# pabloconrat/our_first_climate_model

Hardware: NVIDIA B200
Metric: column*wavelength*layer flux updates/s (repwvl-100 RCE step) (higher is better)
Workload: dtype f64

## Files before the change

### our_first_climate_model_b200/csrc/rcm_capi.cu

```cuda
#include <algorithm>
#include <cmath>
#include <cstdio>
#include <cstdlib>
#include <cstring>
#include <new>
#include <functional>
#include <string>
#include <vector>

#include "rcm_jac.cuh"
#include "rcm_fdh.cuh"

#ifndef M_PI
#define M_PI 3.14159265358979323846
#endif

struct rcm_solver {
    int device = 0;
    cudaStream_t own_stream = nullptr, stream = nullptr;
    rcm_params p{};
    DevConst dc{};
    bool const_dirty = true;
    int opt_angle_cubes = 1;
    int opt_angle_pairs = 1;
    int opt_config = 0;
    int opt_stage_rows = 1;
    int opt_path = 0;
    int opt_cplk_narrow = 0;
    double tau_clamp = 240.0;
    double T_floor = 0.0;
    int clampk = 1;
    bool has_table = false, has_spectral = false;
    std::vector<double> p_grid, t_ref, t_pert, wvl, weight;
    double* d_coef3 = nullptr;
    double *d_xsec_file = nullptr, *d_coef = nullptr, *d_planck_c = nullptr, *d_planck_k = nullptr, *d_exp_tab = nullptr;
    int* d_species = nullptr;
    bool coef_dirty = true;
    int ncol = 0, cap = 0, nactive = 0, h2o_slot = -1;
    int species[RCM_NSPECIES]{};
    bool has_plevel = false;
    double plevel[RCM_NLEVEL]{};
    double *d_T = nullptr, *d_Ts = nullptr, *d_vmr = nullptr, *d_rh = nullptr, *d_Tprev = nullptr;
    float* d_time = nullptr;
    double *d_Ed = nullptr, *d_Eu = nullptr, *d_dE = nullptr, *d_dt = nullptr;
    double *d_diag = nullptr, *d_scalars = nullptr, *d_tau = nullptr, *d_red = nullptr;
    int* d_lowpos = nullptr;
    unsigned* d_ticket = nullptr;
    double *d_solar_col = nullptr, *d_cloud_col = nullptr;
    bool has_col_solar = false, has_col_cloud = false;
    size_t diag_steps = 0, tau_cap = 0;
    long step_index = 0;
    bool tau_valid = false;
    bool lbl_mode = false;
    int lbl_nwvl = 0;
    double lbl_co2_factor = 1.0;
    bool lbl_has_o3_ref = false;
    double *d_lbl_lo = nullptr, *d_lbl_hi = nullptr, *d_lbl_tau5 = nullptr, *d_lbl_h2o_ref = nullptr,
           *d_lbl_o3_ref = nullptr, *d_sH = nullptr, *d_sO = nullptr, *d_dTstat = nullptr, *d_part = nullptr;
    size_t part_cap = 0;
    unsigned char* d_tile = nullptr;
    double* d_spart = nullptr;
    unsigned* d_counter = nullptr;
    unsigned* d_multi = nullptr;
    size_t multi_cap = 0;
    int opt_multi = 1;
    size_t tile_cap = 0, spart_cap = 0;
    bool tile_vmr_valid = false;
    std::vector<double> stage;
    std::string err;
    long launches = 0;
    std::vector<std::pair<cudaEvent_t, cudaEvent_t>> ev_free, ev_used;
    cudaStream_t pipe_stream[3] = {nullptr, nullptr, nullptr};
    cudaEvent_t pipe_done[3] = {nullptr, nullptr, nullptr}, pipe_start = nullptr;
    struct HostGraph {
        cudaGraphExec_t exec = nullptr;
        SplitArgs sig{};
        const void* host[7] = {};
        const void* dev[4] = {};
        double dT_converged = 0.0;
        int ncol = 0, nchunk = 0, nkernels = 0;
        long captures = 0, replays = 0;
        bool failed = false;
    } hg;
    cudaStream_t sp_up = nullptr, sp_rt[2] = {nullptr, nullptr}, sp_down = nullptr;
    cudaEvent_t sp_prep[24] = {}, sp_rtdone[24] = {}, sp_end = nullptr;
    double kt_ms = 0.0;
    long kt_n = 0;
    unsigned char* d_diagnose = nullptr;
    size_t diagnose_bytes = 0;
    cudaStream_t dg_stream[2] = {nullptr, nullptr};
    cudaEvent_t dg_fork = nullptr, dg_join[2] = {nullptr, nullptr};
    int* h_fdh_count = nullptr;
};

namespace {

int fail(rcm_solver* s, int code, const std::string& msg) {
    if (s) s->err = msg;
    return code;
}

int cuda_fail(rcm_solver* s, cudaError_t e, const char* what) {
    return fail(s, RCM_ERR_CUDA, std::string(what) + ": " + cudaGetErrorString(e));
}

#define CU(call)                                          \
    do {                                                  \
        cudaError_t e__ = (call);                         \
        if (e__ != cudaSuccess) return cuda_fail(s, e__, #call); \
    } while (0)

template <class T>
cudaError_t dalloc(T*& p, size_t n) {
    if (p) cudaFree(p);
    p = nullptr;
    return cudaMalloc((void**)&p, n * sizeof(T));
}

void set_active_species(rcm_solver* s) {
    s->nactive = 0;
    s->h2o_slot = -1;
    for (int k = 0; k < RCM_NSPECIES; ++k)
        if (s->p.species_mask & (1u << k)) {
            if (k == 0) s->h2o_slot = s->nactive;
            s->species[s->nactive++] = k;
        }
}

void build_angles(rcm_solver* s) {
    DevConst& d = s->dc;
    const int na = s->p.nangle;
    const double dmu = 1.0 / (double)na;
    d.nangle = na;
    std::vector<std::vector<int>> chains;
    struct PairUnit { int type; double inv_mu_root; std::vector<int> a, b; };
    std::vector<PairUnit> pairs;
    if (s->opt_angle_cubes) {
        std::vector<char> used(na, 0);
        for (int i = na - 1; i >= 0; --i) {
            if (used[i]) continue;
            std::vector<int> ch;
            for (int n = 2 * i + 1;; n /= 3) {
                used[(n - 1) / 2] = 1;
                ch.push_back((n - 1) / 2);
                if (n % 3 != 0) break;
            }
            chains.push_back(ch);
        }
        if (s->opt_angle_pairs) {
            struct Edge { int ca, cb, type, R; };
            std::vector<Edge> edges;
            const int pa_[3] = {3, 5, 3}, pb_[3] = {5, 7, 7};
            for (size_t x = 0; x < chains.size(); ++x)
                for (size_t y = 0; y < chains.size(); ++y) {
                    const int a = 2 * chains[x][0] + 1, b = 2 * chains[y][0] + 1;
                    for (int t = 0; t < 3; ++t)
                        if (a > b && pa_[t] * a == pb_[t] * b) edges.push_back({(int)x, (int)y, t, pa_[t] * a});
                }
            std::vector<int> best, cur;
            std::vector<char> taken(chains.size(), 0);
            std::function<void(size_t)> rec = [&](size_t e) {
                if (cur.size() > best.size()) best = cur;
                if (e >= edges.size() || cur.size() + (edges.size() - e) <= best.size() || edges.size() > 24) return;
                if (!taken[edges[e].ca] && !taken[edges[e].cb]) {
                    taken[edges[e].ca] = taken[edges[e].cb] = 1;
                    cur.push_back((int)e);
                    rec(e + 1);
                    cur.pop_back();
                    taken[edges[e].ca] = taken[edges[e].cb] = 0;
                }
                rec(e + 1);
            };
            rec(0);
            if (best.size() > (size_t)MAX_PAIR) best.resize(MAX_PAIR);
            std::vector<char> gone(chains.size(), 0);
            for (int e : best) {
                const Edge& ed = edges[e];
                pairs.push_back({ed.type, 2.0 * na / (double)ed.R, chains[ed.ca], chains[ed.cb]});
                gone[ed.ca] = gone[ed.cb] = 1;
            }
            std::vector<std::vector<int>> rest;
            for (size_t x = 0; x < chains.size(); ++x)
                if (!gone[x]) rest.push_back(chains[x]);
            chains.swap(rest);
        }
    } else {
        for (int i = 0; i < na; ++i) chains.push_back({i});
    }
    if (chains.size() % 2) chains.push_back({-1});
    d.nchain = (int)chains.size();
    double sum = 0.0, x_max = 0.0, x_min = 1e300;
    int slot = 0;
    for (int a = 0; a < MAX_ANGLE + 2; ++a) {
        d.chain_len[a] = 1;
        d.neg_inv_mu_l2e[a] = 0.0;
        d.cmu[a] = 0.0;
    }
    auto node_mu = [&](int i) { return dmu / 2.0 + dmu * (double)i; };
    d.npair = (int)pairs.size();
    for (int p = 0; p <= MAX_PAIR; ++p) d.pair_nim[p] = 0.0;
    for (int p = 0; p < d.npair; ++p) {
        d.pair_type[p] = pairs[p].type;
        d.pair_lenA[p] = (int)pairs[p].a.size();
        d.pair_lenB[p] = (int)pairs[p].b.size();
        d.pair_nim[p] = -pairs[p].inv_mu_root * EXP_L2E;
        x_max = std::max(x_max, pairs[p].inv_mu_root);
        for (const std::vector<int>* ch : {&pairs[p].a, &pairs[p].b})
            for (int i : *ch) {
                const double mu = node_mu(i);
                d.cmu[slot] = 2 * M_PI * mu * dmu;
                sum += d.cmu[slot++];
                x_min = std::min(x_min, 1.0 / mu);
            }
    }
    for (int ic = 0; ic < d.nchain; ++ic) {
        d.chain_len[ic] = (int)chains[ic].size();
        for (size_t m = 0; m < chains[ic].size(); ++m, ++slot) {
            if (chains[ic][m] < 0) continue;
            const double mu = node_mu(chains[ic][m]);
            d.cmu[slot] = 2 * M_PI * mu * dmu;
            sum += d.cmu[slot];
            if (m == 0) {
                d.neg_inv_mu_l2e[ic] = (-1.0 / mu) * EXP_L2E;
                x_max = std::max(x_max, 1.0 / mu);
            }
            x_min = std::min(x_min, 1.0 / mu);
        }
    }
    d.pair_nim[d.npair] = d.neg_inv_mu_l2e[0];
    d.nslot = slot;
    d.csum = sum;
    {
        const double ec7[4] = {0x1.62e42fefa3685p-8, 0x1.ebfbdff82c58fp-17, 0x1.c6b09b1799fcbp-26, 0x1.3b2ab6fba4e77p-35};
        const double ec10[4] = {0x1.62e42fefa39efp-11, 0x1.ebfbe033445b4p-23, 0x1.c6b08d704a0c0p-35, 0.0};
        for (int k = 0; k < 4; ++k) d.expc[k] = (EXP_LOG2 == 7) ? ec7[k] : ec10[k];
#ifdef RCM_EXP_DEG_OVERRIDE
        {
            const double c = 0.6931471805599453 / EXP_TAB;
            const double tay[4] = {c, c * c / 2, c * c * c / 6, c * c * c * c / 24};
            for (int k = 0; k < 4; ++k) d.expc[k] = (k <= EXP_DEG) ? tay[k] : 0.0;
        }
#endif
    }
    s->tau_clamp = 999.0 * 0.6931471805599453 / x_max;
    s->clampk = (s->tau_clamp * x_min > 92.2) ? 0 : 1;
}

const rcm_solver* g_const_owner[64] = {nullptr};

int refresh_const(rcm_solver* s) {
    const int dev = s->device & 63;
    if (g_const_owner[dev] != s) {
        CU(cudaDeviceSynchronize());
        s->const_dirty = true;
        g_const_owner[dev] = s;
    }
    if (!s->const_dirty) return RCM_OK;
    CU(cudaStreamSynchronize(s->stream));
    DevConst& d = s->dc;
    set_active_species(s);
    d.nactive = s->nactive;
    for (int k = 0; k < RCM_NSPECIES; ++k) d.species[k] = (k < s->nactive) ? s->species[k] : 0;
    d.cloud_layer = s->p.cloud_layer;
    d.cloud_row = s->p.cloud_layer < 0 ? -1 : (s->p.cloud_layer < HALF ? s->p.cloud_layer : 29 - s->p.cloud_layer);
    d.cloud_tau = s->p.cloud_tau;
    for (int r = 0; r < RCM_NLAYER; ++r) d.cloud_w[r] = (r == d.cloud_row) ? 1.0 : 0.0;
    d.dp = s->p.dp;
    d.max_dT = s->p.max_dT;
    d.dt_cap = s->p.dt_cap;
    d.solar_irr = s->p.solar_irr;
    d.dT_converged = s->p.dT_converged;
    build_angles(s);
    if (s->has_table && s->has_plevel) {
        const double avog = 6.02214076e23, molMassAir = 0.0289647, earthAccel = 9.80665;
        double P[RCM_NLEVEL];
        for (int k = 0; k < RCM_NLEVEL; ++k) P[k] = s->plevel[RCM_NLEVEL - 1 - k] * 100.0;
        for (int k = 0; k < RCM_NLAYER; ++k) {
            const int l = RCM_NLAYER - 1 - k;
            const int r = l < HALF ? l : 29 - l;
            const double midP = (P[k + 1] + P[k]) / 2;
            const long ip = rcm_lowerpos_impl(s->p_grid.data(), (int)s->p_grid.size(), midP);
            d.ip[l] = (int)ip;
            d.ipcell[r] = r * (d.n_tpert - 1);
            d.delP[r] = (midP - s->p_grid[ip]) / (s->p_grid[ip + 1] - s->p_grid[ip]);
            d.numDens[r] = (P[k] - P[k + 1]) * avog / molMassAir / earthAccel;
            d.tref_ip[r] = s->t_ref[ip];
        }
    }
    if (s->has_plevel) {
        for (int l = 0; l < RCM_NLAYER; ++l) {
            d.player[l] = (s->plevel[l] + s->plevel[l + 1]) / 2.0;
            d.conv[l] = std::pow(1000.0 / d.player[l], 2.0 / 7.0);
        }
    }
    cudaError_t e = rcm_upload_const(d);
    if (e != cudaSuccess) return cuda_fail(s, e, "upload constants");
    if (s->has_table && s->has_plevel && s->coef_dirty) {
        const size_t n = (size_t)RCM_NLAYER * (d.n_tpert - 1) * d.nwvl * s->nactive * 4;
        CU(dalloc(s->d_coef, n));
        CU(dalloc(s->d_species, (size_t)RCM_NSPECIES));
        CU(cudaMemcpyAsync(s->d_species, s->species, sizeof(s->species), cudaMemcpyHostToDevice, s->stream));
        CU(rcm_launch_coef(s->d_xsec_file, s->d_coef, d.n_tpert, d.n_species, d.nwvl, d.n_p, s->nactive, s->d_species,
                           s->stream));
        if (s->nactive == 5) {
            const size_t nrows = (size_t)RCM_NLAYER * (d.n_tpert - 1) * d.nwvl;
            CU(dalloc(s->d_coef3, nrows * 16));
            CU(rcm_launch_coef3(s->d_coef, s->d_coef3, nrows, s->stream));
            s->launches += 1;
        }
        CU(cudaStreamSynchronize(s->stream));
        s->launches += 1;
        s->coef_dirty = false;
    }
    s->const_dirty = false;
    return RCM_OK;
}

int ensure_columns(rcm_solver* s, int ncol) {
    if (ncol <= s->cap && s->d_T) return RCM_OK;
    const size_t n = (size_t)ncol;
    CU(dalloc(s->d_T, n * NLAY));
    CU(dalloc(s->d_Ts, n));
    CU(dalloc(s->d_vmr, n * RCM_NSPECIES * NLAY));
    CU(dalloc(s->d_rh, n * NLAY));
    CU(dalloc(s->d_Tprev, n * NLAY));
    CU(dalloc(s->d_time, n));
    CU(dalloc(s->d_Ed, n * NLEV));
    CU(dalloc(s->d_Eu, n * NLEV));
    CU(dalloc(s->d_dE, n * NLAY));
    CU(dalloc(s->d_dt, n));
    CU(dalloc(s->d_lowpos, n * NLAY));
    s->cap = ncol;
    s->diag_steps = 0;
    s->part_cap = 0;
    s->tile_cap = s->spart_cap = 0;
    s->tile_vmr_valid = false;
    if (s->d_dTstat) cudaFree(s->d_dTstat);
    s->d_dTstat = nullptr;
    if (s->d_solar_col) cudaFree(s->d_solar_col);
    if (s->d_cloud_col) cudaFree(s->d_cloud_col);
    s->d_solar_col = s->d_cloud_col = nullptr;
    s->has_col_solar = s->has_col_cloud = false;
    return RCM_OK;
}

int ensure_diag(rcm_solver* s, int nsteps) {
    if ((size_t)nsteps <= s->diag_steps && s->d_diag) return RCM_OK;
    CU(dalloc(s->d_diag, (size_t)nsteps * s->cap * 4));
    CU(dalloc(s->d_scalars, (size_t)nsteps * 4));
    CU(dalloc(s->d_red, rcm_reduce_scratch_doubles(nsteps)));
    CU(dalloc(s->d_ticket, (size_t)nsteps));
    CU(cudaMemsetAsync(s->d_ticket, 0, (size_t)nsteps * sizeof(unsigned), s->stream));
    s->diag_steps = nsteps;
    return RCM_OK;
}

int ensure_tau(rcm_solver* s) {
    const size_t need = (size_t)s->ncol * s->dc.nwvl * NLAY;
    if (need <= s->tau_cap && s->d_tau) return RCM_OK;
    CU(dalloc(s->d_tau, need));
    s->tau_cap = need;
    return RCM_OK;
}

struct CtaShape { int C, nthreads, per_sm; double eff; };
const CtaShape kShapes[] = {{16, 128, 3, 1.0}, {8, 128, 3, 0.95}, {4, 128, 3, 0.89}, {32, 192, 2, 0.9}, {16, 96, 4, 0.93}};
constexpr int kAutoShapes = 3;

struct Part { int col0, ncols; CtaShape sh; };

double part_cost(const CtaShape& sh, int ncols, int nwvl, int nsm) {
    if (ncols <= 0) return 0.0;
    const long tiles = (ncols + sh.C - 1) / sh.C, slots = (long)nsm * sh.per_sm;
    const long rounds = (tiles + slots - 1) / slots;
    const int G = sh.nthreads / (2 * sh.C);
    return (double)rounds * ((nwvl + G - 1) / G) / sh.eff;
}

int plan_parts(const rcm_solver* s, int ncol, int nsm, Part* parts) {
    if (s->opt_config > 0 && s->opt_config <= 5) {
        parts[0] = {0, ncol, kShapes[s->opt_config - 1]};
        return 1;
    }
    const int nwvl = s->dc.nwvl;
    CtaShape best = kShapes[0];
    for (int k = 1; k < kAutoShapes; ++k)
        if (part_cost(kShapes[k], ncol, nwvl, nsm) < part_cost(best, ncol, nwvl, nsm)) best = kShapes[k];
    parts[0] = {0, ncol, best};
    return 1;
}

int nsm_of(const rcm_solver* s) {
    int nsm = 148;
    cudaDeviceGetAttribute(&nsm, cudaDevAttrMultiProcessorCount, s->device);
    return nsm;
}

int launch_part(rcm_solver* s, int mode, int nsteps, bool want_diag, const Part& p, int nsm, cudaStream_t st) {
    const size_t o = (size_t)p.col0;
    StepArgs a{};
    a.ncol = p.ncols;
    a.diag_ncol = s->ncol;
    a.C = p.sh.C;
    a.ntiles = (p.ncols + a.C - 1) / a.C;
    a.nthreads = p.sh.nthreads;
    a.clampk = s->clampk;
    a.stage_rows = s->opt_stage_rows;
    a.tau_clamp = s->tau_clamp;
    a.T_floor = s->T_floor;
    a.nsteps = nsteps;
    a.step_index = s->step_index;
    a.coef = s->d_coef;
    a.planck_c = s->d_planck_c;
    a.planck_k = s->d_planck_k;
    a.Tlayer = s->d_T + o * NLAY;
    a.Tsurf = s->d_Ts + o;
    a.vmr = s->d_vmr + o * s->nactive * NLAY;
    a.rel_hum = s->d_rh + o * NLAY;
    a.Tprev = s->d_Tprev + o * NLAY;
    a.time_h = s->d_time + o;
    a.E_down = s->d_Ed + o * NLEV;
    a.E_up = s->d_Eu + o * NLEV;
    a.dE = s->d_dE + o * NLAY;
    a.dt = s->d_dt + o;
    a.diag = want_diag ? s->d_diag + o * 4 : nullptr;
    a.tau_io = s->d_tau ? s->d_tau + o * s->dc.nwvl * NLAY : nullptr;
    a.lowpos_t = s->d_lowpos + o * NLAY;
    a.exp_tab = s->d_exp_tab;
    a.h2o_slot = s->h2o_slot;
    a.solar_col = s->has_col_solar ? s->d_solar_col + o : nullptr;
    a.cloud_col = s->has_col_cloud ? s->d_cloud_col + o : nullptr;
    int per_sm = p.sh.per_sm;
    if (rcm_step_smem_bytes(a.C, s->nactive, a.nthreads) * per_sm > 224 * 1024) per_sm = 1;
    if (const char* e = std::getenv("RCM_CTAS_PER_SM")) {
        const int v = std::atoi(e);
        if (v >= 1 && v < per_sm) per_sm = v;
    }
    const int ctas = nsm * per_sm;
    const int grid = a.ntiles < ctas ? a.ntiles : ctas;
    CU(rcm_launch_step(mode, a, s->nactive, grid, st));
    s->launches += 1;
    return RCM_OK;
}


bool use_split(const rcm_solver* s) {
    return !s->lbl_mode && s->has_table && s->nactive == 5 && s->opt_config == 0 && s->opt_path == 0;
}

struct SplitGeom { int ntiles, nitem, nsplit; };
SplitGeom split_geom(const rcm_solver* s, int ncols) {
    SplitGeom g;
    g.ntiles = (ncols + 15) / 16;
    g.nitem = (s->dc.nwvl + 3) / 4;
    g.nsplit = (g.nitem + rcm_split_ipu() - 1) / rcm_split_ipu();
    return g;
}

int ensure_split(rcm_solver* s) {
    const SplitGeom g = split_geom(s, s->cap);
    const size_t tiles = (size_t)g.ntiles, need_part = tiles * g.nsplit * rcm_split_part_doubles();
    if (tiles > s->tile_cap || !s->d_tile) {
        CU(dalloc(s->d_tile, tiles * rcm_split_tile_bytes()));
        s->tile_cap = tiles;
        s->tile_vmr_valid = false;
    }
    if (need_part > s->spart_cap || !s->d_spart) {
        CU(dalloc(s->d_spart, need_part));
        s->spart_cap = need_part;
    }
    if (tiles > s->multi_cap || !s->d_multi) {
        if (s->d_multi) CU(cudaFree(s->d_multi));
        s->d_multi = nullptr;
        CU(cudaMalloc((void**)&s->d_multi, 2 * tiles * sizeof(unsigned)));
        s->multi_cap = tiles;
    }
    if (!s->d_dTstat) CU(dalloc(s->d_dTstat, (size_t)s->cap));
    if (!s->d_counter) {
        CU(dalloc(s->d_counter, (size_t)4));
        CU(cudaMemsetAsync(s->d_counter, 0, 4 * sizeof(unsigned), s->stream));
    }
    return RCM_OK;
}

SplitArgs split_args(rcm_solver* s, int col0, int ncols, int which) {
    const SplitGeom g = split_geom(s, ncols);
    const size_t o = (size_t)col0, t0 = o / 16;
    SplitArgs a{};
    a.ncol = ncols;
    a.diag_ncol = s->ncol;
    a.ntiles = g.ntiles;
    a.nsplit = g.nsplit;
    a.ipu = rcm_split_ipu();
    a.nitem = g.nitem;
    a.nunits = g.ntiles * g.nsplit;
    a.stage_rows = s->opt_stage_rows;
    a.clampk = s->clampk;
    a.h2o_slot = s->h2o_slot;
    a.tau_clamp = s->tau_clamp;
    a.T_floor = s->T_floor;
    a.coef = s->d_coef3;
    a.planck_c = s->d_planck_c;
    a.planck_k = s->d_planck_k;
    a.exp_tab = s->d_exp_tab;
    a.Tlayer = s->d_T + o * NLAY;
    a.Tsurf = s->d_Ts + o;
    a.vmr = s->d_vmr + o * s->nactive * NLAY;
    a.rel_hum = s->d_rh + o * NLAY;
    a.Tprev = s->d_Tprev + o * NLAY;
    a.time_h = s->d_time + o;
    a.E_down = s->d_Ed + o * NLEV;
    a.E_up = s->d_Eu + o * NLEV;
    a.dE = s->d_dE + o * NLAY;
    a.dt = s->d_dt + o;
    a.diag = s->d_diag + o * 4;
    a.solar_col = s->has_col_solar ? s->d_solar_col + o : nullptr;
    a.cloud_col = s->has_col_cloud ? s->d_cloud_col + o : nullptr;
    a.tile = s->d_tile + t0 * rcm_split_tile_bytes();
    a.part = s->d_spart + t0 * g.nsplit * rcm_split_part_doubles();
    a.dTstat = s->d_dTstat + o;
    a.counter = s->d_counter + which;
    a.quota = 1 << 30;
    return a;
}

int split_grid(const rcm_solver* s, const SplitArgs& a, int nsm) {
    (void)s;
    if (a.quota < a.nunits) return (a.nunits + a.quota - 1) / a.quota;
    int per_sm = 3;
    if (const char* e = std::getenv("RCM_CTAS_PER_SM")) {
        const int v = std::atoi(e);
        if (v >= 1 && v < per_sm) per_sm = v;
    }
    return std::min(a.nunits, nsm * per_sm);
}

int split_rt(rcm_solver* s, const SplitArgs& a, int nsm, cudaStream_t st, bool timed) {
    std::pair<cudaEvent_t, cudaEvent_t> ev{};
    if (timed) {
        if (!s->ev_free.empty()) {
            ev = s->ev_free.back();
            s->ev_free.pop_back();
        } else {
            CU(cudaEventCreate(&ev.first));
            CU(cudaEventCreate(&ev.second));
        }
        CU(cudaEventRecord(ev.first, st));
    }
    CU(rcm_launch_split_rt(a, split_grid(s, a, nsm), st));
    s->launches += 1;
    if (timed) {
        CU(cudaEventRecord(ev.second, st));
        s->ev_used.push_back(ev);
        if (s->ev_used.size() >= 1024) {
            const int rc = rcm_kernel_time_ms(s, 0, nullptr, nullptr);
            if (rc != RCM_OK) return rc;
        }
    }
    return RCM_OK;
}

int split_advance(rcm_solver* s, int nsteps) {
    int st = refresh_const(s);
    if (st != RCM_OK) return st;
    st = ensure_split(s);
    if (st != RCM_OK) return st;
    const int nsm = nsm_of(s);
    const SplitArgs a = split_args(s, 0, s->ncol, 0);
    SplitColFlags f{};
    f.prep = 1;
    f.first = (s->step_index == 0);
    f.write_all_vmr = !s->tile_vmr_valid;
    CU(rcm_launch_split_col(a, f, s->stream));
    s->launches += 1;
    s->tile_vmr_valid = true;
    static const int multi_rounds = std::getenv("RCM_MULTI_ROUNDS") ? std::atoi(std::getenv("RCM_MULTI_ROUNDS")) : 24;
    const int grid1 = split_grid(s, a, nsm);
    const bool few_rounds = a.nunits < (long long)multi_rounds * grid1;
    const bool fits = (long long)a.nunits * nsteps + 2LL * grid1 < (1LL << 31);
    if (nsteps >= 2 && fits && (s->opt_multi == 2 || (s->opt_multi == 1 && few_rounds))) {
        SplitMultiArgs m{};
        m.nsteps = nsteps;
        m.done = s->d_multi;
        m.ready = s->d_multi + a.ntiles;
        CU(cudaMemsetAsync(s->d_multi, 0, 2 * (size_t)a.ntiles * sizeof(unsigned), s->stream));
        SplitArgs am = a;
        am.quota = 1 << 30;
        CU(rcm_launch_split_multi(am, m, split_grid(s, am, nsm), s->stream));
        s->launches += 1;
        return RCM_OK;
    }
    for (int k = 0; k < nsteps; ++k) {
        st = split_rt(s, a, nsm, s->stream, k < 4);
        if (st != RCM_OK) return st;
        SplitColFlags e{};
        e.finish = 1;
        e.prep = (k + 1 < nsteps);
        e.first = 0;
        e.write_out = (k + 1 == nsteps);
        e.diag_step = k;
        CU(rcm_launch_split_col(a, e, s->stream));
        s->launches += 1;
    }
    return RCM_OK;
}

int launch(rcm_solver* s, int mode, int nsteps, bool want_diag) {
    int st = refresh_const(s);
    if (st != RCM_OK) return st;
    if (mode == MODE_RT ? !s->has_spectral : !s->has_table) return fail(s, RCM_ERR_STATE, "no lookup table loaded");
    if (s->ncol <= 0) return fail(s, RCM_ERR_STATE, "no columns loaded");
    const int nsm = nsm_of(s);
    Part parts[2];
    const int nparts = plan_parts(s, s->ncol, nsm, parts);
    std::pair<cudaEvent_t, cudaEvent_t> ev;
    if (!s->ev_free.empty()) {
        ev = s->ev_free.back();
        s->ev_free.pop_back();
    } else {
        CU(cudaEventCreate(&ev.first));
        CU(cudaEventCreate(&ev.second));
    }
    CU(cudaEventRecord(ev.first, s->stream));
    for (int ip = 0; ip < nparts; ++ip) {
        st = launch_part(s, mode, nsteps, want_diag, parts[ip], nsm, s->stream);
        if (st != RCM_OK) return st;
    }
    CU(cudaEventRecord(ev.second, s->stream));
    if (mode == MODE_STEP) s->ev_used.push_back(ev); else s->ev_free.push_back(ev);
    if (s->ev_used.size() >= 1024) {
        st = rcm_kernel_time_ms(s, 0, nullptr, nullptr);
        if (st != RCM_OK) return st;
    }
    return RCM_OK;
}


int step_host_split(rcm_solver* s, int nchunk, const double* Tlayer_in, const double* Tsurf_in, const double* vmr_active_in,
                    double* E_down, double* E_up, double* dE, double* Tlayer_out, double* Tsurf_out) {
    int st = ensure_split(s);
    if (st != RCM_OK) return st;
    if (!s->sp_up) {
        int lo = 0, hi = 0;
        CU(cudaDeviceGetStreamPriorityRange(&lo, &hi));
        CU(cudaStreamCreateWithPriority(&s->sp_up, cudaStreamNonBlocking, hi));
        CU(cudaStreamCreateWithPriority(&s->sp_down, cudaStreamNonBlocking, hi));
        for (int i = 0; i < 2; ++i) CU(cudaStreamCreateWithPriority(&s->sp_rt[i], cudaStreamNonBlocking, lo));
        for (int i = 0; i < 24; ++i) {
            CU(cudaEventCreateWithFlags(&s->sp_prep[i], cudaEventDisableTiming));
            CU(cudaEventCreateWithFlags(&s->sp_rtdone[i], cudaEventDisableTiming));
        }
        CU(cudaEventCreateWithFlags(&s->sp_end, cudaEventDisableTiming));
    }
    const int nsm = nsm_of(s);
    const int per = ((s->ncol + nchunk - 1) / nchunk + 15) / 16 * 16;
    int bounds[24];
    int nb = 0;
    bounds[nb++] = 0;
    if (nchunk >= 4 && per >= 64) {
        const int q = per / 4 / 16 * 16;
        bounds[nb++] = q;
        for (int c0 = per; c0 < s->ncol - q; c0 += per) bounds[nb++] = c0;
        bounds[nb++] = std::max(bounds[nb - 1], s->ncol - q) / 16 * 16;
    } else {
        for (int c0 = per; c0 < s->ncol; c0 += per) bounds[nb++] = c0;
    }
    bounds[nb] = s->ncol;
    const size_t D = sizeof(double);
    const int na = s->nactive;
    auto enqueue = [&](bool timed) -> int {
    int nk = 0;
    CU(cudaEventRecord(s->sp_end, s->stream));
    for (cudaStream_t q : {s->sp_up, s->sp_rt[0], s->sp_rt[1], s->sp_down}) CU(cudaStreamWaitEvent(q, s->sp_end, 0));
    for (int k = 0; k < nb; ++k) {
        const int c0 = bounds[k], n = bounds[k + 1] - c0;
        if (n <= 0) continue;
        const size_t o = (size_t)c0;
        cudaStream_t q = s->sp_up;
        if (Tlayer_in) CU(cudaMemcpyAsync(s->d_T + o * NLAY, Tlayer_in + o * NLAY, n * NLAY * D, cudaMemcpyHostToDevice, q));
        if (Tsurf_in) CU(cudaMemcpyAsync(s->d_Ts + o, Tsurf_in + o, n * D, cudaMemcpyHostToDevice, q));
        if (vmr_active_in)
            CU(cudaMemcpyAsync(s->d_vmr + o * na * NLAY, vmr_active_in + o * na * NLAY, (size_t)n * na * NLAY * D,
                               cudaMemcpyHostToDevice, q));
        SplitArgs a = split_args(s, c0, n, 1 + k % 2);
        a.quota = 4;
        SplitArgs ac = a;
        ac.counter = nullptr;
        SplitColFlags f{};
        f.prep = 1;
        f.first = (s->step_index == 0);
        f.write_all_vmr = !s->tile_vmr_valid || vmr_active_in != nullptr;
        CU(rcm_launch_split_col(ac, f, q));
        CU(cudaEventRecord(s->sp_prep[k], q));
        q = s->sp_rt[k % 2];
        CU(cudaStreamWaitEvent(q, s->sp_prep[k], 0));
        CU(cudaMemsetAsync(a.counter, 0, sizeof(unsigned), q));
        st = split_rt(s, a, nsm, q, timed);
        if (st != RCM_OK) return st;
        nk += 3;
        CU(cudaEventRecord(s->sp_rtdone[k], q));
        q = s->sp_down;
        CU(cudaStreamWaitEvent(q, s->sp_rtdone[k], 0));
        SplitColFlags e{};
        e.finish = 1;
        e.write_out = 1;
        CU(rcm_launch_split_col(ac, e, q));
        s->launches += 2;
        if (E_down) CU(cudaMemcpyAsync(E_down + o * NLEV, s->d_Ed + o * NLEV, n * NLEV * D, cudaMemcpyDeviceToHost, q));
        if (E_up) CU(cudaMemcpyAsync(E_up + o * NLEV, s->d_Eu + o * NLEV, n * NLEV * D, cudaMemcpyDeviceToHost, q));
        if (dE) CU(cudaMemcpyAsync(dE + o * NLAY, s->d_dE + o * NLAY, n * NLAY * D, cudaMemcpyDeviceToHost, q));
        if (Tlayer_out) CU(cudaMemcpyAsync(Tlayer_out + o * NLAY, s->d_T + o * NLAY, n * NLAY * D, cudaMemcpyDeviceToHost, q));
        if (Tsurf_out) CU(cudaMemcpyAsync(Tsurf_out + o, s->d_Ts + o, n * D, cudaMemcpyDeviceToHost, q));
    }
    CU(cudaEventRecord(s->sp_end, s->sp_down));
    CU(cudaStreamWaitEvent(s->stream, s->sp_end, 0));
    CU(rcm_launch_reduce_diag(s->d_diag, 1, s->ncol, s->p.dT_converged, s->d_red, s->d_ticket, s->d_scalars, s->stream));
    s->launches += 1;
    s->hg.nkernels = nk + 1;
    return RCM_OK;
    };

    const bool steady = s->step_index > 0 && s->tile_vmr_valid && !vmr_active_in && !s->hg.failed && !std::getenv("RCM_NO_GRAPH");
    bool launched = false;
    if (steady) {
        rcm_solver::HostGraph& g = s->hg;
        const SplitArgs sig = split_args(s, 0, s->ncol, 1);
        const void* host[7] = {Tlayer_in, Tsurf_in, E_down, E_up, dE, Tlayer_out, Tsurf_out};
        const void* dev[4] = {s->d_diag, s->d_red, s->d_ticket, s->d_scalars};
        const bool same = g.exec && std::memcmp(&g.sig, &sig, sizeof(sig)) == 0 && std::memcmp(g.host, host, sizeof(host)) == 0 &&
                          std::memcmp(g.dev, dev, sizeof(dev)) == 0 && g.dT_converged == s->p.dT_converged && g.ncol == s->ncol &&
                          g.nchunk == nchunk;
        if (!same) {
            if (g.exec) cudaGraphExecDestroy(g.exec);
            g.exec = nullptr;
            cudaGraph_t graph = nullptr;
            const long launches0 = s->launches;
            bool ok = true;
            for (const void* hp : host) {
                cudaPointerAttributes at{};
                if (hp && (cudaPointerGetAttributes(&at, hp) != cudaSuccess || at.type != cudaMemoryTypeHost)) ok = false;
            }
            cudaGetLastError();
            ok = ok && cudaStreamBeginCapture(s->stream, cudaStreamCaptureModeRelaxed) == cudaSuccess;
            if (ok) {
                ok = enqueue(false) == RCM_OK;
                ok = (cudaStreamEndCapture(s->stream, &graph) == cudaSuccess) && ok && graph;
            }
            s->launches = launches0;
            g.captures += 1;
            if (ok) ok = cudaGraphInstantiate(&g.exec, graph, 0) == cudaSuccess;
            if (graph) cudaGraphDestroy(graph);
            if (!ok) {
                cudaGetLastError();
                g.exec = nullptr;
                bool pinned = true;
                for (const void* hp : host) {
                    cudaPointerAttributes at{};
                    if (hp && (cudaPointerGetAttributes(&at, hp) != cudaSuccess || at.type != cudaMemoryTypeHost)) pinned = false;
                }
                cudaGetLastError();
                if (pinned) g.failed = true;
            } else {
                g.sig = sig;
                std::memcpy(g.host, host, sizeof(host));
                std::memcpy(g.dev, dev, sizeof(dev));
                g.dT_converged = s->p.dT_converged;
                g.ncol = s->ncol;
                g.nchunk = nchunk;
            }
        }
        if (g.exec) {
            CU(cudaGraphLaunch(g.exec, s->stream));
            s->launches += g.nkernels;
            g.replays += 1;
            launched = true;
        }
    }
    if (!launched) {
        st = enqueue(true);
        if (st != RCM_OK) return st;
    }
    s->step_index += 1;
    s->tau_valid = false;
    s->tile_vmr_valid = true;
    CU(cudaStreamSynchronize(s->stream));
    return RCM_OK;
}

}

extern "C" {

int rcm_device_count(void) {
    int n = 0;
    if (cudaGetDeviceCount(&n) != cudaSuccess) return 0;
    return n;
}

int rcm_create(int device, const rcm_params* p, rcm_solver** out) {
    if (!out) return RCM_ERR_ARG;
    *out = nullptr;
    int n = 0;
    if (cudaGetDeviceCount(&n) != cudaSuccess || n <= 0) return RCM_ERR_NO_DEVICE;
    if (device < 0 || device >= n) return RCM_ERR_ARG;
    rcm_solver* s = new (std::nothrow) rcm_solver();
    if (!s) return RCM_ERR_NOMEM;
    s->device = device;
    if (p) s->p = *p; else rcm_default_params(&s->p);
    if (s->p.nangle < 1 || s->p.nangle > MAX_ANGLE || s->p.cloud_layer >= RCM_NLAYER) {
        delete s;
        return RCM_ERR_ARG;
    }
    if (cudaSetDevice(device) != cudaSuccess || cudaStreamCreateWithFlags(&s->own_stream, cudaStreamNonBlocking) != cudaSuccess) {
        delete s;
        return RCM_ERR_CUDA;
    }
    s->stream = s->own_stream;
    double tab[EXP_TAB];
    for (int j = 0; j < EXP_TAB; ++j) {
        const double v = std::exp2((double)j / EXP_TAB);
        unsigned long long bits;
        std::memcpy(&bits, &v, 8);
        bits -= (unsigned long long)j << (20 - EXP_LOG2 + 32);
        std::memcpy(&tab[j], &bits, 8);
    }
    if (dalloc(s->d_exp_tab, EXP_TAB) != cudaSuccess ||
        cudaMemcpy(s->d_exp_tab, tab, sizeof(tab), cudaMemcpyHostToDevice) != cudaSuccess) {
        delete s;
        return RCM_ERR_CUDA;
    }
    set_active_species(s);
    *out = s;
    return RCM_OK;
}

int rcm_destroy(rcm_solver* s) {
    if (!s) return RCM_OK;
    cudaSetDevice(s->device);
    cudaStreamSynchronize(s->stream);
    if (g_const_owner[s->device & 63] == s) g_const_owner[s->device & 63] = nullptr;
    void* ptrs[] = {s->d_coef3, s->d_xsec_file, s->d_coef, s->d_species, s->d_planck_c, s->d_planck_k, s->d_exp_tab, s->d_T, s->d_Ts, s->d_vmr, s->d_rh,
                    s->d_Tprev, s->d_time, s->d_lbl_lo, s->d_lbl_hi, s->d_lbl_tau5, s->d_lbl_h2o_ref, s->d_lbl_o3_ref, s->d_sH, s->d_sO,
                    s->d_dTstat, s->d_part, s->d_Ed, s->d_Eu, s->d_dE, s->d_dt, s->d_diag, s->d_scalars, s->d_red, s->d_tau,
                    s->d_lowpos, s->d_solar_col, s->d_cloud_col, s->d_ticket, s->d_tile, s->d_spart, s->d_counter, s->d_multi, s->d_diagnose};
    for (void* q : ptrs)
        if (q) cudaFree(q);
    for (auto& e : s->ev_free) { cudaEventDestroy(e.first); cudaEventDestroy(e.second); }
    for (auto& e : s->ev_used) { cudaEventDestroy(e.first); cudaEventDestroy(e.second); }
    for (int i = 0; i < 3; ++i) {
        if (s->pipe_stream[i]) cudaStreamDestroy(s->pipe_stream[i]);
        if (s->pipe_done[i]) cudaEventDestroy(s->pipe_done[i]);
    }
    if (s->pipe_start) cudaEventDestroy(s->pipe_start);
    for (cudaStream_t q : {s->sp_up, s->sp_rt[0], s->sp_rt[1], s->sp_down})
        if (q) cudaStreamDestroy(q);
    for (int i = 0; i < 24; ++i) {
        if (s->sp_prep[i]) cudaEventDestroy(s->sp_prep[i]);
        if (s->sp_rtdone[i]) cudaEventDestroy(s->sp_rtdone[i]);
    }
    if (s->sp_end) cudaEventDestroy(s->sp_end);
    for (int i = 0; i < 2; ++i) {
        if (s->dg_stream[i]) cudaStreamDestroy(s->dg_stream[i]);
        if (s->dg_join[i]) cudaEventDestroy(s->dg_join[i]);
    }
    if (s->dg_fork) cudaEventDestroy(s->dg_fork);
    if (s->h_fdh_count) cudaFreeHost(s->h_fdh_count);
    if (s->hg.exec) cudaGraphExecDestroy(s->hg.exec);
    if (s->own_stream) cudaStreamDestroy(s->own_stream);
    delete s;
    return RCM_OK;
}

const char* rcm_last_error(const rcm_solver* s) { return s ? s->err.c_str() : "null solver"; }

int rcm_set_params(rcm_solver* s, const rcm_params* p) {
    if (!s || !p) return RCM_ERR_ARG;
    if (p->nangle < 1 || p->nangle > MAX_ANGLE || p->cloud_layer >= RCM_NLAYER) return fail(s, RCM_ERR_ARG, "bad params");
    unsigned old = s->p.species_mask;
    s->p = *p;
    if (old != p->species_mask) {
        s->coef_dirty = true;
        s->ncol = 0;
    }
    s->const_dirty = true;
    set_active_species(s);
    return RCM_OK;
}

int rcm_set_option(rcm_solver* s, int option, int value) {
    if (!s) return RCM_ERR_ARG;
    if (option == 0) {
        s->opt_angle_cubes = value ? 1 : 0;
        s->const_dirty = true;
        return RCM_OK;
    }
    if (option == 1) {
        s->opt_config = value;
        s->tile_vmr_valid = false;
        return RCM_OK;
    }
    if (option == 2) {
        s->opt_cplk_narrow = value ? 1 : 0;
        return RCM_OK;
    }
    if (option == 3) {
        s->opt_stage_rows = value ? 1 : 0;
        return RCM_OK;
    }
    if (option == 4) {
        s->opt_angle_pairs = value ? 1 : 0;
        s->const_dirty = true;
        return RCM_OK;
    }
    if (option == 5) {
        s->opt_path = value ? 1 : 0;
        s->tile_vmr_valid = false;
        return RCM_OK;
    }
    if (option == 6) {
        s->opt_multi = value < 0 ? 0 : value > 2 ? 2 : value;
        return RCM_OK;
    }
    return fail(s, RCM_ERR_ARG, "unknown option");
}

int rcm_set_stream(rcm_solver* s, void* cuda_stream) {
    if (!s) return RCM_ERR_ARG;
    s->stream = cuda_stream ? (cudaStream_t)cuda_stream : s->own_stream;
    return RCM_OK;
}

int rcm_synchronize(rcm_solver* s) {
    if (!s) return RCM_ERR_ARG;
    CU(cudaSetDevice(s->device));
    CU(cudaStreamSynchronize(s->stream));
    return RCM_OK;
}

int rcm_set_repwvl_table(rcm_solver* s, const double* xsec, const double* wvl, const double* weight,
                         const double* p_grid, const double* t_ref, const double* t_pert, int n_tpert, int n_species,
                         int n_wvl, int n_p) {
    if (!s || !xsec || !wvl || !weight || !p_grid || !t_ref || !t_pert) return RCM_ERR_ARG;
    if (n_tpert < 2 || n_tpert > MAX_TPERT || n_species != RCM_NSPECIES || n_wvl < 1 || n_p < 2)
        return fail(s, RCM_ERR_ARG, "unsupported table dimensions");
    CU(cudaSetDevice(s->device));
    const size_t n = (size_t)n_tpert * n_species * n_wvl * n_p;
    CU(dalloc(s->d_xsec_file, n));
    CU(cudaMemcpy(s->d_xsec_file, xsec, n * sizeof(double), cudaMemcpyHostToDevice));
    s->coef_dirty = true;
    {
        int st = rcm_set_spectral_grid(s, wvl, weight, n_wvl);
        if (st != RCM_OK) return st;
    }
    s->p_grid.assign(p_grid, p_grid + n_p);
    s->t_ref.assign(t_ref, t_ref + n_p);
    s->t_pert.assign(t_pert, t_pert + n_tpert);
    s->dc.nwvl = n_wvl;
    s->dc.n_tpert = n_tpert;
    s->dc.n_species = n_species;
    s->dc.n_p = n_p;
    for (int m = 0; m < n_tpert; ++m) s->dc.t_pert[m] = t_pert[m];
    s->has_table = true;
    s->lbl_mode = false;
    s->const_dirty = true;
    s->tau_valid = false;
    s->tau_cap = 0;
    return RCM_OK;
}

int rcm_set_spectral_grid(rcm_solver* s, const double* wvl, const double* weight, int n_wvl) {
    if (!s || !wvl || !weight || n_wvl < 1) return RCM_ERR_ARG;
    CU(cudaSetDevice(s->device));
    const double h = 6.62607e-34, c = 299792458, kB = 1.380649e-23;
    std::vector<double> pc(n_wvl), pk(n_wvl);
    double pc_max = 0.0;
    for (int i = 0; i < n_wvl; ++i) {
        const double lam = wvl[i] * 1e-9;
        pc[i] = h * c / (lam * kB);
        pk[i] = weight[i] * 2 * h * std::pow(c, 2) / std::pow(lam, 5) / 1e9;
        if (!(wvl[i] > 0.0) || !std::isfinite(pk[i])) return fail(s, RCM_ERR_ARG, "wavelengths must be positive and finite");
        pc_max = std::max(pc_max, pc[i]);
    }
    if (pc_max / 690.0 > 20.0)
        return fail(s, RCM_ERR_ARG, "wavelengths below 1043 nm are not supported (thermal solver: the Planck exponent would leave the range of the kernels' exp)");
    s->T_floor = pc_max / 690.0;
    CU(dalloc(s->d_planck_c, (size_t)n_wvl));
    CU(dalloc(s->d_planck_k, (size_t)n_wvl));
    CU(cudaMemcpy(s->d_planck_c, pc.data(), n_wvl * sizeof(double), cudaMemcpyHostToDevice));
    CU(cudaMemcpy(s->d_planck_k, pk.data(), n_wvl * sizeof(double), cudaMemcpyHostToDevice));
    s->wvl.assign(wvl, wvl + n_wvl);
    s->weight.assign(weight, weight + n_wvl);
    if (s->dc.nwvl != n_wvl) {
        s->has_table = false;
        s->tau_cap = 0;
    }
    s->dc.nwvl = n_wvl;
    s->has_spectral = true;
    s->lbl_mode = false;
    s->const_dirty = true;
    s->tau_valid = false;
    return RCM_OK;
}

int rcm_set_repwvl_table_from(rcm_solver* s, const rcm_table* t) {
    if (!s || !t) return RCM_ERR_ARG;
    return rcm_set_repwvl_table(s, t->xsec.data(), t->wvl.data(), t->weight.data(), t->p_grid.data(), t->t_ref.data(),
                                t->t_pert.data(), t->n_tpert, t->n_species, t->n_wvl, t->n_p);
}

int rcm_set_lbl_tables(rcm_solver* s, const double* wvl, const double* tau5, int nwvl, const double* h2o_ref,
                       const double* o3_ref, double co2_factor) {
    if (!s || !wvl || !tau5 || nwvl < 2 || !h2o_ref) return RCM_ERR_ARG;
    for (int i = 1; i < nwvl; ++i)
        if (!(wvl[i] > wvl[i - 1])) return fail(s, RCM_ERR_ARG, "LBL wavelengths must be strictly ascending");
    CU(cudaSetDevice(s->device));
    std::vector<double> lo(nwvl), hi(nwvl);
    for (int i = 0; i < nwvl; ++i) {
        const double dl = (i > 0) ? (wvl[i] - wvl[i - 1]) : (wvl[1] - wvl[0]);
        const double dh = (i < nwvl - 1) ? (wvl[i + 1] - wvl[i]) : (wvl[i] - wvl[i - 1]);
        lo[i] = wvl[i] - dl / 2.0;
        hi[i] = wvl[i] + dh / 2.0;
    }
    const size_t n = (size_t)nwvl;
    CU(dalloc(s->d_lbl_lo, 4 * n));
    CU(dalloc(s->d_lbl_hi, n));
    CU(dalloc(s->d_lbl_tau5, 3 * n * NLAY));
    CU(dalloc(s->d_lbl_h2o_ref, (size_t)NLAY));
    CU(dalloc(s->d_lbl_o3_ref, (size_t)NLAY));
    CU(cudaMemcpy(s->d_lbl_lo, lo.data(), n * sizeof(double), cudaMemcpyHostToDevice));
    {
        std::vector<double> wn(2 * n);
        std::vector<int> ok(2 * n, 0);
        for (size_t i = 0; i < n; ++i) {
            const double whi = 1.0E7 / lo[i], wlo = 1.0E7 / hi[i];
            wn[i] = whi;
            wn[n + i] = wlo;
            ok[i] = (whi > wlo && wlo >= 0. && (whi - wlo) / whi < 1.e-2) ? 1 : 0;
        }
        CU(cudaMemcpy(s->d_lbl_lo + n, wn.data(), 2 * n * sizeof(double), cudaMemcpyHostToDevice));
        CU(cudaMemcpy(s->d_lbl_lo + 3 * n, ok.data(), n * sizeof(int), cudaMemcpyHostToDevice));
    }
    CU(cudaMemcpy(s->d_lbl_hi, hi.data(), n * sizeof(double), cudaMemcpyHostToDevice));
    {
        const size_t plane = n * NLAY;
        std::vector<double> t3(3 * plane);
        std::memcpy(&t3[0], tau5, plane * sizeof(double));
        std::memcpy(&t3[plane], tau5 + 2 * plane, plane * sizeof(double));
        for (size_t i = 0; i < plane; ++i) t3[2 * plane + i] = co2_factor * tau5[plane + i] + tau5[3 * plane + i] + tau5[4 * plane + i];
        CU(cudaMemcpy(s->d_lbl_tau5, t3.data(), t3.size() * sizeof(double), cudaMemcpyHostToDevice));
    }
    CU(cudaMemcpy(s->d_lbl_h2o_ref, h2o_ref, NLAY * sizeof(double), cudaMemcpyHostToDevice));
    s->lbl_has_o3_ref = o3_ref != nullptr;
    if (o3_ref) CU(cudaMemcpy(s->d_lbl_o3_ref, o3_ref, NLAY * sizeof(double), cudaMemcpyHostToDevice));
    s->lbl_nwvl = nwvl;
    s->lbl_co2_factor = co2_factor;
    s->lbl_mode = true;
    if (s->dc.nwvl != nwvl) {
        s->has_table = s->has_spectral = false;
        s->tau_cap = 0;
    }
    s->tau_valid = false;
    s->dc.nwvl = nwvl;
    s->const_dirty = true;
    s->part_cap = 0;
    return RCM_OK;
}

int rcm_set_columns(rcm_solver* s, int ncol, const double* plevel_hPa, const double* Tlayer, const double* Tsurf,
                    const double* vmr9, const double* rel_hum) {
    if (!s || ncol <= 0 || !plevel_hPa || !Tlayer || !Tsurf || !vmr9 || !rel_hum) return RCM_ERR_ARG;
    CU(cudaSetDevice(s->device));
    int st = ensure_columns(s, ncol);
    if (st != RCM_OK) return st;
    s->ncol = ncol;
    if (!s->has_plevel || std::memcmp(s->plevel, plevel_hPa, sizeof(s->plevel)) != 0) s->coef_dirty = true;
    std::memcpy(s->plevel, plevel_hPa, sizeof(s->plevel));
    s->has_plevel = true;
    s->const_dirty = true;
    set_active_species(s);
    const size_t n = (size_t)ncol;
    s->stage.resize(n * s->nactive * NLAY);
    for (size_t c = 0; c < n; ++c)
        for (int k = 0; k < s->nactive; ++k)
            std::memcpy(&s->stage[(c * s->nactive + k) * NLAY], vmr9 + (c * RCM_NSPECIES + s->species[k]) * NLAY,
                        NLAY * sizeof(double));
    CU(cudaMemcpyAsync(s->d_vmr, s->stage.data(), s->stage.size() * sizeof(double), cudaMemcpyHostToDevice, s->stream));
    CU(cudaMemcpyAsync(s->d_T, Tlayer, n * NLAY * sizeof(double), cudaMemcpyHostToDevice, s->stream));
    CU(cudaMemcpyAsync(s->d_Tprev, Tlayer, n * NLAY * sizeof(double), cudaMemcpyHostToDevice, s->stream));
    CU(cudaMemcpyAsync(s->d_Ts, Tsurf, n * sizeof(double), cudaMemcpyHostToDevice, s->stream));
    CU(cudaMemcpyAsync(s->d_rh, rel_hum, n * NLAY * sizeof(double), cudaMemcpyHostToDevice, s->stream));
    CU(cudaMemsetAsync(s->d_time, 0, n * sizeof(float), s->stream));
    CU(cudaStreamSynchronize(s->stream));
    s->step_index = 0;
    s->tau_valid = false;
    s->tile_vmr_valid = false;
    s->has_col_solar = s->has_col_cloud = false;
    return RCM_OK;
}

int rcm_set_column_solar(rcm_solver* s, const rcm_solar_params* sp, const double* tau_s, const double* mu_s,
                         const double* albedo, int cloud_from_tau_s, double* solar_irr_out, double* r_total_out) {
    if (!s) return RCM_ERR_ARG;
    if (s->ncol <= 0) return fail(s, RCM_ERR_STATE, "rcm_set_columns first");
    CU(cudaSetDevice(s->device));
    if (!sp) {
        s->has_col_solar = s->has_col_cloud = false;
        s->tau_valid = false;
        return RCM_OK;
    }
    if (sp->doublings < 0 || sp->doublings > 60) return fail(s, RCM_ERR_ARG, "doublings must be in 0..60");
    if (cloud_from_tau_s && s->p.cloud_layer < 0) return fail(s, RCM_ERR_ARG, "cloud_from_tau_s needs a cloud layer");
    const size_t n = (size_t)s->ncol;
    if (!s->d_solar_col) {
        CU(dalloc(s->d_solar_col, (size_t)s->cap));
        CU(dalloc(s->d_cloud_col, (size_t)s->cap));
    }
    double* d_in = nullptr;
    CU(cudaMalloc((void**)&d_in, 3 * n * sizeof(double)));
    const double* src[3] = {tau_s, mu_s, albedo};
    for (int k = 0; k < 3; ++k)
        if (src[k]) {
            cudaError_t e = cudaMemcpyAsync(d_in + k * n, src[k], n * sizeof(double), cudaMemcpyHostToDevice, s->stream);
            if (e != cudaSuccess) { cudaFree(d_in); return cuda_fail(s, e, "upload solar inputs"); }
        }
    double* d_rt = nullptr;
    if (r_total_out) {
        cudaError_t e = cudaMalloc((void**)&d_rt, n * sizeof(double));
        if (e != cudaSuccess) { cudaFree(d_in); return cuda_fail(s, e, "cudaMalloc"); }
    }
    SolarArgs a{};
    a.n = s->ncol;
    a.doublings = sp->doublings;
    a.tau_s = sp->tau_s; a.mu_s = sp->mu_s; a.g_asym = sp->g_asym; a.albedo = sp->albedo; a.daytime = sp->daytime; a.E_0 = sp->E_0;
    a.tau_s_col = tau_s ? d_in : nullptr;
    a.mu_s_col = mu_s ? d_in + n : nullptr;
    a.albedo_col = albedo ? d_in + 2 * n : nullptr;
    a.solar_irr = s->d_solar_col;
    a.r_total = d_rt;
    a.cloud_tau = cloud_from_tau_s ? s->d_cloud_col : nullptr;
    cudaError_t e = rcm_launch_solar(a, s->stream);
    if (e == cudaSuccess && solar_irr_out)
        e = cudaMemcpyAsync(solar_irr_out, s->d_solar_col, n * sizeof(double), cudaMemcpyDeviceToHost, s->stream);
    if (e == cudaSuccess && r_total_out)
        e = cudaMemcpyAsync(r_total_out, d_rt, n * sizeof(double), cudaMemcpyDeviceToHost, s->stream);
    if (e == cudaSuccess) e = cudaStreamSynchronize(s->stream);
    cudaFree(d_in);
    if (d_rt) cudaFree(d_rt);
    if (e != cudaSuccess) return cuda_fail(s, e, "rcm_set_column_solar");
    s->launches += 1;
    s->has_col_solar = true;
    s->has_col_cloud = cloud_from_tau_s != 0;
    s->tau_valid = false;
    return RCM_OK;
}

int rcm_update_columns(rcm_solver* s, const double* Tlayer, const double* Tsurf, const double* vmr_active) {
    if (!s) return RCM_ERR_ARG;
    if (s->ncol <= 0) return fail(s, RCM_ERR_STATE, "rcm_set_columns first");
    CU(cudaSetDevice(s->device));
    const size_t n = (size_t)s->ncol;
    if (Tlayer) CU(cudaMemcpyAsync(s->d_T, Tlayer, n * NLAY * sizeof(double), cudaMemcpyHostToDevice, s->stream));
    if (Tsurf) CU(cudaMemcpyAsync(s->d_Ts, Tsurf, n * sizeof(double), cudaMemcpyHostToDevice, s->stream));
    if (vmr_active)
        CU(cudaMemcpyAsync(s->d_vmr, vmr_active, n * s->nactive * NLAY * sizeof(double), cudaMemcpyHostToDevice, s->stream));
    if (vmr_active) s->tile_vmr_valid = false;
    s->tau_valid = false;
    return RCM_OK;
}

int rcm_set_step_index(rcm_solver* s, long step_index) {
    if (!s || step_index < 0) return RCM_ERR_ARG;
    s->step_index = step_index;
    return RCM_OK;
}

int rcm_build_tau(rcm_solver* s, double* tau_out, int* lowpos_p, int* lowpos_t) {
    if (!s) return RCM_ERR_ARG;
    if (s->lbl_mode) return fail(s, RCM_ERR_STATE, "rcm_build_tau is the repwvl read_tau: set a repwvl table after rcm_set_lbl_tables");
    if (!s->has_table || s->ncol <= 0) return fail(s, RCM_ERR_STATE, "table and columns must be loaded");
    CU(cudaSetDevice(s->device));
    int st = ensure_tau(s);
    if (st != RCM_OK) return st;
    st = launch(s, MODE_TAU, 1, false);
    if (st != RCM_OK) return st;
    const size_t n = (size_t)s->ncol;
    if (tau_out)
        CU(cudaMemcpyAsync(tau_out, s->d_tau, n * s->dc.nwvl * NLAY * sizeof(double), cudaMemcpyDeviceToHost, s->stream));
    std::vector<int> lt;
    if (lowpos_t) CU(cudaMemcpyAsync(lowpos_t, s->d_lowpos, n * NLAY * sizeof(int), cudaMemcpyDeviceToHost, s->stream));
    CU(cudaStreamSynchronize(s->stream));
    if (lowpos_p)
        for (size_t c = 0; c < n; ++c)
            for (int k = 0; k < NLAY; ++k) lowpos_p[c * NLAY + k] = s->dc.ip[NLAY - 1 - k];
    s->tau_valid = true;
    return RCM_OK;
}

int rcm_radiative_transfer(rcm_solver* s, const double* tau, double* E_down, double* E_up, double* dE) {
    if (!s) return RCM_ERR_ARG;
    if (s->lbl_mode) return fail(s, RCM_ERR_STATE, "rcm_radiative_transfer needs a repwvl spectral grid: set one after rcm_set_lbl_tables");
    if (!s->has_spectral || s->ncol <= 0) return fail(s, RCM_ERR_STATE, "spectral grid and columns must be loaded");
    CU(cudaSetDevice(s->device));
    int st = ensure_tau(s);
    if (st != RCM_OK) return st;
    const size_t n = (size_t)s->ncol;
    if (tau) {
        CU(cudaMemcpyAsync(s->d_tau, tau, n * s->dc.nwvl * NLAY * sizeof(double), cudaMemcpyHostToDevice, s->stream));
    } else if (!s->tau_valid) {
        return fail(s, RCM_ERR_STATE, "no tau: pass one or call rcm_build_tau first");
    }
    st = launch(s, MODE_RT, 1, false);
    if (st != RCM_OK) return st;
    if (E_down) CU(cudaMemcpyAsync(E_down, s->d_Ed, n * NLEV * sizeof(double), cudaMemcpyDeviceToHost, s->stream));
    if (E_up) CU(cudaMemcpyAsync(E_up, s->d_Eu, n * NLEV * sizeof(double), cudaMemcpyDeviceToHost, s->stream));
    if (dE) CU(cudaMemcpyAsync(dE, s->d_dE, n * NLAY * sizeof(double), cudaMemcpyDeviceToHost, s->stream));
    CU(cudaStreamSynchronize(s->stream));
    return RCM_OK;
}

static int lbl_advance(rcm_solver* s, int nsteps) {
    if (s->h2o_slot < 0) return fail(s, RCM_ERR_STATE, "the LBL path needs H2O in species_mask");
    int st = refresh_const(s);
    if (st != RCM_OK) return st;
    const size_t n = (size_t)s->ncol;
    if (!s->d_sH || s->part_cap == 0) {
        CU(dalloc(s->d_sH, (size_t)s->cap * NLAY));
        CU(dalloc(s->d_sO, (size_t)s->cap * NLAY));
        CU(dalloc(s->d_dTstat, (size_t)s->cap));
    }
    LblArgs a{};
    a.ncol = s->ncol;
    a.ntiles = (s->ncol + RCM_LBL_C - 1) / RCM_LBL_C;
    a.nwvl = s->lbl_nwvl;
    a.chunk_len = 128;
    a.nchunks = (a.nwvl + a.chunk_len - 1) / a.chunk_len;
    const size_t need = (size_t)a.nchunks * n * 42;
    if (need > s->part_cap) {
        CU(dalloc(s->d_part, need));
        s->part_cap = need;
    }
    a.nact = s->nactive;
    a.h2o_slot = s->h2o_slot;
    a.o3_slot = -1;
    for (int k = 0; k < s->nactive; ++k)
        if (s->species[k] == 2) a.o3_slot = k;
    a.co2_factor = s->lbl_co2_factor;
    a.clampk = s->clampk;
    a.tau_clamp = s->tau_clamp;
    a.wvl_lo = s->d_lbl_lo;
    a.wvl_hi = s->d_lbl_hi;
    a.wn_hi = s->d_lbl_lo + (size_t)s->lbl_nwvl;
    a.wn_lo = s->d_lbl_lo + 2 * (size_t)s->lbl_nwvl;
    a.bin_ok = reinterpret_cast<const int*>(s->d_lbl_lo + 3 * (size_t)s->lbl_nwvl);
    a.tau3 = s->d_lbl_tau5;
    a.h2o_ref = s->d_lbl_h2o_ref;
    a.o3_ref = s->lbl_has_o3_ref ? s->d_lbl_o3_ref : nullptr;
    a.exp_tab = s->d_exp_tab;
    a.Tlayer = s->d_T; a.Tsurf = s->d_Ts; a.vmr = s->d_vmr; a.rel_hum = s->d_rh; a.Tprev = s->d_Tprev;
    a.time_h = s->d_time; a.sH = s->d_sH; a.sO = s->d_sO; a.dTstat = s->d_dTstat; a.part = s->d_part;
    a.E_down = s->d_Ed; a.E_up = s->d_Eu; a.dE = s->d_dE; a.dt = s->d_dt;
    a.solar_col = s->has_col_solar ? s->d_solar_col : nullptr;
    a.cloud_col = s->has_col_cloud ? s->d_cloud_col : nullptr;
    for (int k = 0; k < nsteps; ++k) {
        a.step_index = s->step_index + k;
        a.diag = s->d_diag + (size_t)k * s->ncol * 4;
        std::pair<cudaEvent_t, cudaEvent_t> ev{};
        if (!s->ev_free.empty()) {
            ev = s->ev_free.back();
            s->ev_free.pop_back();
        } else {
            CU(cudaEventCreate(&ev.first));
            CU(cudaEventCreate(&ev.second));
        }
        CU(rcm_launch_lbl_step(a, s->stream, ev.first, ev.second));
        s->ev_used.push_back(ev);
        if (s->ev_used.size() >= 1024) {
            st = rcm_kernel_time_ms(s, 0, nullptr, nullptr);
            if (st != RCM_OK) return st;
        }
        s->launches += 3;
    }
    return RCM_OK;
}

int rcm_advance_async(rcm_solver* s, int nsteps, double** d_scalars) {
    if (!s || nsteps <= 0) return RCM_ERR_ARG;
    if ((!s->has_table && !s->lbl_mode) || s->ncol <= 0) return fail(s, RCM_ERR_STATE, "table and columns must be loaded");
    CU(cudaSetDevice(s->device));
    int st = ensure_diag(s, nsteps);
    if (st != RCM_OK) return st;
    if (s->lbl_mode) {
        st = lbl_advance(s, nsteps);
        if (st != RCM_OK) return st;
        CU(rcm_launch_reduce_diag(s->d_diag, nsteps, s->ncol, s->p.dT_converged, s->d_red, s->d_ticket, s->d_scalars, s->stream));
        s->launches += 1;
        s->step_index += nsteps;
        if (d_scalars) *d_scalars = s->d_scalars;
        return RCM_OK;
    }
    st = use_split(s) ? split_advance(s, nsteps) : launch(s, MODE_STEP, nsteps, true);
    if (st != RCM_OK) return st;
    CU(rcm_launch_reduce_diag(s->d_diag, nsteps, s->ncol, s->p.dT_converged, s->d_red, s->d_ticket, s->d_scalars, s->stream));
    s->launches += 1;
    s->step_index += nsteps;
    s->tau_valid = false;
    if (d_scalars) *d_scalars = s->d_scalars;
    return RCM_OK;
}

int rcm_advance(rcm_solver* s, int nsteps, rcm_step_scalars* scalars_out) {
    int st = rcm_advance_async(s, nsteps, nullptr);
    if (st != RCM_OK) return st;
    if (scalars_out) {
        CU(cudaMemcpyAsync(scalars_out, s->d_scalars, (size_t)nsteps * sizeof(rcm_step_scalars), cudaMemcpyDeviceToHost,
                           s->stream));
        CU(cudaStreamSynchronize(s->stream));
    }
    return RCM_OK;
}

int rcm_run_to_equilibrium(rcm_solver* s, long max_steps, int check_every, rcm_step_scalars* last, long* steps_done) {
    if (!s || max_steps <= 0 || check_every <= 0) return RCM_ERR_ARG;
    if (steps_done) *steps_done = 0;
    std::vector<rcm_step_scalars> sc((size_t)check_every);
    long done = 0;
    while (done < max_steps) {
        const int n = (int)std::min<long>(check_every, max_steps - done);
        const int st = rcm_advance(s, n, sc.data());
        if (st != RCM_OK) return st;
        done += n;
        if (last) *last = sc[n - 1];
        if (steps_done) *steps_done = done;
        if (sc[n - 1].n_converged >= (double)s->ncol) break;
    }
    return RCM_OK;
}

int rcm_get_state(rcm_solver* s, double* Tlayer, double* Tsurf, double* h2o, float* time_h, double* E_down,
                  double* E_up, double* dE, double* dt) {
    if (!s) return RCM_ERR_ARG;
    if (s->ncol <= 0) return fail(s, RCM_ERR_STATE, "no columns loaded");
    CU(cudaSetDevice(s->device));
    const size_t n = (size_t)s->ncol;
    if (Tlayer) CU(cudaMemcpyAsync(Tlayer, s->d_T, n * NLAY * sizeof(double), cudaMemcpyDeviceToHost, s->stream));
    if (Tsurf) CU(cudaMemcpyAsync(Tsurf, s->d_Ts, n * sizeof(double), cudaMemcpyDeviceToHost, s->stream));
    if (time_h) CU(cudaMemcpyAsync(time_h, s->d_time, n * sizeof(float), cudaMemcpyDeviceToHost, s->stream));
    if (E_down) CU(cudaMemcpyAsync(E_down, s->d_Ed, n * NLEV * sizeof(double), cudaMemcpyDeviceToHost, s->stream));
    if (E_up) CU(cudaMemcpyAsync(E_up, s->d_Eu, n * NLEV * sizeof(double), cudaMemcpyDeviceToHost, s->stream));
    if (dE) CU(cudaMemcpyAsync(dE, s->d_dE, n * NLAY * sizeof(double), cudaMemcpyDeviceToHost, s->stream));
    if (dt) CU(cudaMemcpyAsync(dt, s->d_dt, n * sizeof(double), cudaMemcpyDeviceToHost, s->stream));
    if (h2o) {
        if (s->h2o_slot < 0) return fail(s, RCM_ERR_STATE, "H2O is not an active species");
        CU(cudaMemcpy2DAsync(h2o, NLAY * sizeof(double), s->d_vmr + (size_t)s->h2o_slot * NLAY,
                             (size_t)s->nactive * NLAY * sizeof(double), NLAY * sizeof(double), n, cudaMemcpyDeviceToHost,
                             s->stream));
    }
    CU(cudaStreamSynchronize(s->stream));
    return RCM_OK;
}

namespace {

constexpr int kDiagMaxChunk = 8192;

int diag_check(rcm_solver* s, const std::string& fn, int col0, int ncol, const double* vmr_scale, DiagScale& sc) {
    if (s->lbl_mode) return fail(s, RCM_ERR_STATE, fn + ": the line-by-line path is not supported");
    if (!s->has_table) return fail(s, RCM_ERR_STATE, fn + ": no lookup table loaded");
    if (s->ncol <= 0) return fail(s, RCM_ERR_STATE, fn + ": no columns loaded");
    if (s->nactive != 5) return fail(s, RCM_ERR_STATE, fn + ": needs the five active species of the default species_mask");
    if (!use_split(s)) return fail(s, RCM_ERR_STATE, fn + ": needs the split path (RCM_OPT_PATH 0, no forced tile shape)");
    if (col0 < 0 || ncol <= 0 || (long long)col0 + ncol > s->ncol)
        return fail(s, RCM_ERR_ARG, fn + ": columns [" + std::to_string(col0) + ", " + std::to_string((long long)col0 + ncol) +
                                        ") outside the " + std::to_string(s->ncol) + " loaded");
    for (int k = 0; k < 5; ++k) {
        sc.f[k] = vmr_scale ? vmr_scale[k] : 1.0;
        if (!(sc.f[k] >= 0.0) || !std::isfinite(sc.f[k]))
            return fail(s, RCM_ERR_ARG, fn + ": vmr_scale[" + std::to_string(k) + "] must be finite and >= 0");
    }
    return RCM_OK;
}

int diag_begin(rcm_solver* s, size_t set_bytes) {
    if (2 * set_bytes > s->diagnose_bytes) {
        CU(dalloc(s->d_diagnose, 2 * set_bytes));
        s->diagnose_bytes = 2 * set_bytes;
    }
    if (!s->dg_fork) {
        for (int i = 0; i < 2; ++i) {
            CU(cudaStreamCreateWithFlags(&s->dg_stream[i], cudaStreamNonBlocking));
            CU(cudaEventCreateWithFlags(&s->dg_join[i], cudaEventDisableTiming));
        }
        CU(cudaEventCreateWithFlags(&s->dg_fork, cudaEventDisableTiming));
    }
    CU(cudaEventRecord(s->dg_fork, s->stream));
    for (int i = 0; i < 2; ++i) CU(cudaStreamWaitEvent(s->dg_stream[i], s->dg_fork, 0));
    return RCM_OK;
}

int diag_prep(rcm_solver* s, cudaStream_t q, int c0, int n, double* dT, double* dTprev, double* dvmr, double* dstat,
              unsigned char* dtile, const DiagScale* sc, SplitArgs& a) {
    constexpr size_t D = sizeof(double);
    const size_t o = (size_t)c0;
    const int na = s->nactive;
    CU(cudaMemcpyAsync(dT, s->d_T + o * NLAY, n * NLAY * D, cudaMemcpyDeviceToDevice, q));
    CU(cudaMemcpyAsync(dTprev, s->d_Tprev + o * NLAY, n * NLAY * D, cudaMemcpyDeviceToDevice, q));
    CU(cudaMemcpyAsync(dvmr, s->d_vmr + o * na * NLAY, (size_t)n * na * NLAY * D, cudaMemcpyDeviceToDevice, q));
    a = split_args(s, c0, n, 0);
    a.Tlayer = dT;
    a.Tprev = dTprev;
    a.vmr = dvmr;
    a.dTstat = dstat;
    a.tile = dtile;
    a.counter = nullptr;
    a.part = nullptr;
    a.diag = nullptr;
    a.E_down = a.E_up = a.dE = a.dt = nullptr;
    a.time_h = nullptr;
    SplitColFlags f{};
    f.prep = 1;
    f.first = (s->step_index == 0);
    f.write_all_vmr = 1;
    CU(rcm_launch_split_col(a, f, q));
    if (sc) CU(rcm_launch_diag_scale(dtile, a.ntiles, *sc, q));
    s->launches += sc ? 2 : 1;
    return RCM_OK;
}

int diag_end(rcm_solver* s) {
    for (int i = 0; i < 2; ++i) {
        CU(cudaEventRecord(s->dg_join[i], s->dg_stream[i]));
        CU(cudaStreamWaitEvent(s->stream, s->dg_join[i], 0));
    }
    CU(cudaStreamSynchronize(s->stream));
    return RCM_OK;
}

}

int rcm_diagnose_fluxes(rcm_solver* s, int col0, int ncol, const double* vmr_scale, double* E_down_spec, double* E_up_spec,
                        double* E_down, double* E_up, double* dE) {
    if (!s) return RCM_ERR_ARG;
    DiagScale sc{};
    int st = diag_check(s, "rcm_diagnose_fluxes", col0, ncol, vmr_scale, sc);
    if (st != RCM_OK) return st;
    CU(cudaSetDevice(s->device));
    st = refresh_const(s);
    if (st != RCM_OK) return st;
    const int nwvl = s->dc.nwvl, na = s->nactive;
    const size_t ch = (size_t)std::min(kDiagMaxChunk, (ncol + 15) / 16 * 16), D = sizeof(double);
    const size_t n_dbl = ch * (2 * NLAY + (size_t)na * NLAY + 1 + 2 * NLEV + NLAY) + 2 * ch * nwvl * NLEV;
    const size_t tile_off = (n_dbl * D + 255) / 256 * 256, set_bytes = (tile_off + ch / 16 * rcm_split_tile_bytes() + 255) / 256 * 256;
    if ((st = diag_begin(s, set_bytes)) != RCM_OK) return st;
    const bool scaled = vmr_scale != nullptr;
    const int nsm = nsm_of(s);
    struct Pending { cudaStream_t q; size_t r; int n; const double *dn, *up, *Ed, *Eu, *dE; } pend{};
    auto download = [&](const Pending& c) -> int {
        const size_t nspec = (size_t)c.n * nwvl * NLEV;
        if (E_down_spec) CU(cudaMemcpyAsync(E_down_spec + c.r * nwvl * NLEV, c.dn, nspec * D, cudaMemcpyDeviceToHost, c.q));
        if (E_up_spec) CU(cudaMemcpyAsync(E_up_spec + c.r * nwvl * NLEV, c.up, nspec * D, cudaMemcpyDeviceToHost, c.q));
        if (E_down) CU(cudaMemcpyAsync(E_down + c.r * NLEV, c.Ed, c.n * NLEV * D, cudaMemcpyDeviceToHost, c.q));
        if (E_up) CU(cudaMemcpyAsync(E_up + c.r * NLEV, c.Eu, c.n * NLEV * D, cudaMemcpyDeviceToHost, c.q));
        if (dE) CU(cudaMemcpyAsync(dE + c.r * NLAY, c.dE, c.n * NLAY * D, cudaMemcpyDeviceToHost, c.q));
        return RCM_OK;
    };
    for (int c0 = col0, k = 0; c0 < col0 + ncol; c0 += (int)ch, ++k) {
        const int n = std::min((int)ch, col0 + ncol - c0);
        const size_t r = (size_t)(c0 - col0);
        cudaStream_t q = s->dg_stream[k % 2];
        double* p = reinterpret_cast<double*>(s->d_diagnose + (k % 2) * set_bytes);
        double* dT = p; p += ch * NLAY;
        double* dTprev = p; p += ch * NLAY;
        double* dvmr = p; p += ch * na * NLAY;
        double* dstat = p; p += ch;
        double* dEd = p; p += ch * NLEV;
        double* dEu = p; p += ch * NLEV;
        double* ddE = p; p += ch * NLAY;
        double* dspec_dn = p; p += ch * nwvl * NLEV;
        double* dspec_up = p;
        unsigned char* dtile = s->d_diagnose + (k % 2) * set_bytes + tile_off;
        SplitArgs a;
        if ((st = diag_prep(s, q, c0, n, dT, dTprev, dvmr, dstat, dtile, scaled ? &sc : nullptr, a)) != RCM_OK) return st;
        DiagArgs g{};
        g.ncol = n;
        g.ntiles = a.ntiles;
        g.nsplit = a.nsplit;
        g.ipu = a.ipu;
        g.nitem = a.nitem;
        g.nunits = a.nunits;
        g.clampk = s->clampk;
        g.tau_clamp = s->tau_clamp;
        g.coef = s->d_coef3;
        g.planck_c = s->d_planck_c;
        g.planck_k = s->d_planck_k;
        g.exp_tab = s->d_exp_tab;
        g.tile = dtile;
        g.spec_dn = dspec_dn;
        g.spec_up = dspec_up;
        g.E_down = dEd;
        g.E_up = dEu;
        g.dE = ddE;
        g.solar_col = a.solar_col;
        CU(rcm_launch_diag_rt(g, std::min(g.nunits, 3 * nsm), q));
        CU(rcm_launch_diag_sum(g, q));
        s->launches += 2;
        if (k > 0 && (st = download(pend)) != RCM_OK) return st;
        pend = {q, r, n, dspec_dn, dspec_up, dEd, dEu, ddE};
    }
    if ((st = download(pend)) != RCM_OK) return st;
    return diag_end(s);
}

int rcm_radiative_kernels(rcm_solver* s, int col0, int ncol, const double* vmr_scale, double* K_spec, double* K) {
    if (!s) return RCM_ERR_ARG;
    DiagScale sc{};
    int st = diag_check(s, "rcm_radiative_kernels", col0, ncol, vmr_scale, sc);
    if (st != RCM_OK) return st;
    if (s->h2o_slot != 0) return fail(s, RCM_ERR_STATE, "rcm_radiative_kernels: needs H2O among the active species");
    CU(cudaSetDevice(s->device));
    st = refresh_const(s);
    if (st != RCM_OK) return st;
    const int nwvl = s->dc.nwvl, na = s->nactive;
    const size_t ch = (size_t)std::min(kDiagMaxChunk, (ncol + 15) / 16 * 16), D = sizeof(double);
    const size_t n_dbl = ch * (2 * NLAY + (size_t)na * NLAY + 1 + JAC_NK) + ch * nwvl * JAC_NK;
    const size_t tile_off = (n_dbl * D + 255) / 256 * 256, set_bytes = (tile_off + ch / 16 * rcm_split_tile_bytes() + 255) / 256 * 256;
    if ((st = diag_begin(s, set_bytes)) != RCM_OK) return st;
    const int grid_max = rcm_jac_ctas_per_sm() * nsm_of(s);
    struct Pending { cudaStream_t q; size_t r; int n; const double *Ks, *K; } pend{};
    auto download = [&](const Pending& c) -> int {
        if (K_spec) CU(cudaMemcpyAsync(K_spec + c.r * nwvl * JAC_NK, c.Ks, (size_t)c.n * nwvl * JAC_NK * D, cudaMemcpyDeviceToHost, c.q));
        if (K) CU(cudaMemcpyAsync(K + c.r * JAC_NK, c.K, (size_t)c.n * JAC_NK * D, cudaMemcpyDeviceToHost, c.q));
        return RCM_OK;
    };
    for (int c0 = col0, k = 0; c0 < col0 + ncol; c0 += (int)ch, ++k) {
        const int n = std::min((int)ch, col0 + ncol - c0);
        const size_t r = (size_t)(c0 - col0);
        cudaStream_t q = s->dg_stream[k % 2];
        double* p = reinterpret_cast<double*>(s->d_diagnose + (k % 2) * set_bytes);
        double* dT = p; p += ch * NLAY;
        double* dTprev = p; p += ch * NLAY;
        double* dvmr = p; p += ch * na * NLAY;
        double* dstat = p; p += ch;
        double* dK = p; p += ch * JAC_NK;
        double* dKs = p;
        unsigned char* dtile = s->d_diagnose + (k % 2) * set_bytes + tile_off;
        SplitArgs a;
        if ((st = diag_prep(s, q, c0, n, dT, dTprev, dvmr, dstat, dtile, vmr_scale ? &sc : nullptr, a)) != RCM_OK) return st;
        JacArgs g{};
        g.ncol = n;
        g.ntiles = a.ntiles;
        g.nsplit = a.nsplit;
        g.ipu = a.ipu;
        g.nitem = a.nitem;
        g.nunits = a.nunits;
        g.clampk = s->clampk;
        g.tau_clamp = s->tau_clamp;
        g.T_floor = s->T_floor;
        g.wtau = 2 * M_PI * (1.0 / (double)s->p.nangle);
        g.coef = s->d_coef3;
        g.planck_c = s->d_planck_c;
        g.planck_k = s->d_planck_k;
        g.exp_tab = s->d_exp_tab;
        g.tile = dtile;
        g.T = dT;
        g.Ts = s->d_Ts + c0;
        g.K_spec = dKs;
        g.K = dK;
        CU(rcm_launch_jac_rt(g, std::min(g.nunits, grid_max), q));
        CU(rcm_launch_jac_sum(g, q));
        s->launches += 2;
        if (k > 0 && (st = download(pend)) != RCM_OK) return st;
        pend = {q, r, n, dKs, dK};
    }
    if ((st = download(pend)) != RCM_OK) return st;
    return diag_end(s);
}

int rcm_flux_jacobian(rcm_solver* s, int col0, int ncol, const double* vmr_scale, double* J, double* dE_jac) {
    if (!s) return RCM_ERR_ARG;
    DiagScale sc{};
    int st = diag_check(s, "rcm_flux_jacobian", col0, ncol, vmr_scale, sc);
    if (st != RCM_OK) return st;
    if (s->h2o_slot != 0) return fail(s, RCM_ERR_STATE, "rcm_flux_jacobian: needs H2O among the active species");
    CU(cudaSetDevice(s->device));
    st = refresh_const(s);
    if (st != RCM_OK) return st;
    const int na = s->nactive;
    const size_t ch = (size_t)std::min(kDiagMaxChunk, (ncol + 15) / 16 * 16), D = sizeof(double);
    const size_t n_dbl = ch * (2 * NLAY + (size_t)na * NLAY + 1 + FJAC_NJ + FJAC_NH);
    const size_t tile_off = (n_dbl * D + 255) / 256 * 256, set_bytes = (tile_off + ch / 16 * rcm_split_tile_bytes() + 255) / 256 * 256;
    if ((st = diag_begin(s, set_bytes)) != RCM_OK) return st;
    struct Pending { cudaStream_t q; size_t r; int n; const double *J, *H; } pend{};
    auto download = [&](const Pending& c) -> int {
        if (J) CU(cudaMemcpyAsync(J + c.r * FJAC_NJ, c.J, (size_t)c.n * FJAC_NJ * D, cudaMemcpyDeviceToHost, c.q));
        if (dE_jac) CU(cudaMemcpyAsync(dE_jac + c.r * FJAC_NH, c.H, (size_t)c.n * FJAC_NH * D, cudaMemcpyDeviceToHost, c.q));
        return RCM_OK;
    };
    for (int c0 = col0, k = 0; c0 < col0 + ncol; c0 += (int)ch, ++k) {
        const int n = std::min((int)ch, col0 + ncol - c0);
        const size_t r = (size_t)(c0 - col0);
        cudaStream_t q = s->dg_stream[k % 2];
        double* p = reinterpret_cast<double*>(s->d_diagnose + (k % 2) * set_bytes);
        double* dT = p; p += ch * NLAY;
        double* dTprev = p; p += ch * NLAY;
        double* dvmr = p; p += ch * na * NLAY;
        double* dstat = p; p += ch;
        double* dJ = p; p += ch * FJAC_NJ;
        double* dH = p;
        unsigned char* dtile = s->d_diagnose + (k % 2) * set_bytes + tile_off;
        SplitArgs a;
        if ((st = diag_prep(s, q, c0, n, dT, dTprev, dvmr, dstat, dtile, vmr_scale ? &sc : nullptr, a)) != RCM_OK) return st;
        FjacArgs g{};
        g.ncol = n;
        g.clampk = s->clampk;
        g.tau_clamp = s->tau_clamp;
        g.T_floor = s->T_floor;
        g.wtau = 2 * M_PI * (1.0 / (double)s->p.nangle);
        g.coef = s->d_coef3;
        g.planck_c = s->d_planck_c;
        g.planck_k = s->d_planck_k;
        g.exp_tab = s->d_exp_tab;
        g.tile = dtile;
        g.T = dT;
        g.Ts = s->d_Ts + c0;
        g.J = dJ;
        g.dE_jac = dH;
        CU(rcm_launch_fjac(g, q));
        s->launches += 1;
        if (k > 0 && (st = download(pend)) != RCM_OK) return st;
        pend = {q, r, n, dJ, dH};
    }
    if ((st = download(pend)) != RCM_OK) return st;
    return diag_end(s);
}

int rcm_adjusted_forcing(rcm_solver* s, int col0, int ncol, const double* vmr_scale, const int* ntrop, double tol, int max_iter,
                         double* F, double* dT_adj, double* E_down, double* E_up, int* iters) {
    if (!s) return RCM_ERR_ARG;
    const std::string fn = "rcm_adjusted_forcing";
    DiagScale sc{};
    int st = diag_check(s, fn, col0, ncol, vmr_scale, sc);
    if (st != RCM_OK) return st;
    if (s->h2o_slot != 0) return fail(s, RCM_ERR_STATE, fn + ": needs H2O among the active species");
    if (!ntrop) return fail(s, RCM_ERR_ARG, fn + ": ntrop is NULL");
    for (int c = 0; c < ncol; ++c)
        if (ntrop[c] < 0 || ntrop[c] > FDH_MAXM)
            return fail(s, RCM_ERR_ARG, fn + ": ntrop[" + std::to_string(c) + "] = " + std::to_string(ntrop[c]) + " outside [0, 19]");
    if (!std::isfinite(tol) || !(tol > 0.0)) return fail(s, RCM_ERR_ARG, fn + ": tol must be finite and > 0");
    if (max_iter < 1) return fail(s, RCM_ERR_ARG, fn + ": max_iter must be >= 1");
    CU(cudaSetDevice(s->device));
    st = refresh_const(s);
    if (st != RCM_OK) return st;
    if (!s->h_fdh_count) CU(cudaMallocHost((void**)&s->h_fdh_count, 2 * sizeof(int)));
    const int nwvl = s->dc.nwvl, na = s->nactive, nsm = nsm_of(s);
    const bool first = (s->step_index == 0);
    const size_t ch = (size_t)std::min(kDiagMaxChunk, (ncol + 15) / 16 * 16), D = sizeof(double);
    const size_t n_dbl = ch * (2 * NLAY + (size_t)na * NLAY + 1 + 3 * NLAY + 2 * (2 * NLEV + NLAY) + 4 + 2 * NLEV + FJAC_NJ + FJAC_NH) +
                         2 * ch * nwvl * NLEV;
    const size_t n_int = 2 * ch + 1;
    const size_t tile_off = (n_dbl * D + n_int * sizeof(int) + 255) / 256 * 256,
                 set_bytes = (tile_off + ch / 16 * rcm_split_tile_bytes() + 255) / 256 * 256;
    if ((st = diag_begin(s, set_bytes)) != RCM_OK) return st;
    struct Slot {
        cudaStream_t q;
        int c0 = 0, n = 0, iter = 0;
        bool live = false;
        double *T, *Tprev, *vmr, *stat, *Ttau, *Tp, *dT, *Ed0, *Eu0, *dE0, *Ed, *Eu, *dE, *F, *Edo, *Euo, *J, *H, *spec_dn, *spec_up;
        int *ntrop, *iters, *count;
        unsigned char* tile;
        SplitArgs a;
    } slot[2];
    for (int k = 0; k < 2; ++k) {
        Slot& z = slot[k];
        z.q = s->dg_stream[k];
        double* p = reinterpret_cast<double*>(s->d_diagnose + k * set_bytes);
        z.T = p; p += ch * NLAY;
        z.Tprev = p; p += ch * NLAY;
        z.vmr = p; p += ch * na * NLAY;
        z.stat = p; p += ch;
        z.Ttau = p; p += ch * NLAY;
        z.Tp = p; p += ch * NLAY;
        z.dT = p; p += ch * NLAY;
        z.Ed0 = p; p += ch * NLEV;
        z.Eu0 = p; p += ch * NLEV;
        z.dE0 = p; p += ch * NLAY;
        z.Ed = p; p += ch * NLEV;
        z.Eu = p; p += ch * NLEV;
        z.dE = p; p += ch * NLAY;
        z.F = p; p += ch * 4;
        z.Edo = p; p += ch * NLEV;
        z.Euo = p; p += ch * NLEV;
        z.J = p; p += ch * FJAC_NJ;
        z.H = p; p += ch * FJAC_NH;
        z.spec_dn = p; p += ch * nwvl * NLEV;
        z.spec_up = p; p += ch * nwvl * NLEV;
        int* ip = reinterpret_cast<int*>(p);
        z.ntrop = ip; ip += ch;
        z.iters = ip; ip += ch;
        z.count = ip;
        z.tile = s->d_diagnose + k * set_bytes + tile_off;
    }
    auto evaluate = [&](Slot& z, double* Ed, double* Eu, double* dE) -> int {
        DiagArgs g{};
        g.ncol = z.n;
        g.ntiles = z.a.ntiles;
        g.nsplit = z.a.nsplit;
        g.ipu = z.a.ipu;
        g.nitem = z.a.nitem;
        g.nunits = z.a.nunits;
        g.clampk = s->clampk;
        g.tau_clamp = s->tau_clamp;
        g.coef = s->d_coef3;
        g.planck_c = s->d_planck_c;
        g.planck_k = s->d_planck_k;
        g.exp_tab = s->d_exp_tab;
        g.tile = z.tile;
        g.spec_dn = z.spec_dn;
        g.spec_up = z.spec_up;
        g.E_down = Ed;
        g.E_up = Eu;
        g.dE = dE;
        g.solar_col = z.a.solar_col;
        CU(rcm_launch_diag_rt(g, std::min(g.nunits, 3 * nsm), z.q));
        CU(rcm_launch_diag_sum(g, z.q));
        s->launches += 2;
        return RCM_OK;
    };
    auto fdh_args = [&](const Slot& z) {
        FdhArgs f{};
        f.ncol = z.n;
        f.iter = z.iter;
        f.max_iter = max_iter;
        f.tol = tol;
        f.T_floor = s->T_floor;
        f.tile = z.tile;
        f.Tb = z.T;
        f.Ttau = first ? z.Ttau : z.T;
        f.Tp = z.Tp;
        f.dT = z.dT;
        f.ntrop = z.ntrop;
        f.Ed0 = z.Ed0;
        f.Eu0 = z.Eu0;
        f.dE0 = z.dE0;
        f.Ed = z.Ed;
        f.Eu = z.Eu;
        f.dE = z.dE;
        f.dE_jac = z.H;
        f.iters = z.iters;
        f.F = z.F;
        f.Ed_out = z.Edo;
        f.Eu_out = z.Euo;
        f.nactive = z.count;
        return f;
    };
    auto check = [&](Slot& z, int k) -> int {
        const FdhArgs f = fdh_args(z);
        CU(rcm_launch_fdh_retemper(f, z.q));
        if ((st = evaluate(z, z.Ed, z.Eu, z.dE)) != RCM_OK) return st;
        CU(rcm_launch_fdh_check(f, z.q));
        CU(cudaMemcpyAsync(s->h_fdh_count + k, z.count, sizeof(int), cudaMemcpyDeviceToHost, z.q));
        s->launches += 2;
        return RCM_OK;
    };
    auto newton = [&](Slot& z) -> int {
        FjacArgs g{};
        g.ncol = z.n;
        g.clampk = s->clampk;
        g.tau_clamp = s->tau_clamp;
        g.T_floor = s->T_floor;
        g.wtau = 2 * M_PI * (1.0 / (double)s->p.nangle);
        g.coef = s->d_coef3;
        g.planck_c = s->d_planck_c;
        g.planck_k = s->d_planck_k;
        g.exp_tab = s->d_exp_tab;
        g.tile = z.tile;
        g.T = z.Tp;
        g.Ts = s->d_Ts + z.c0;
        g.J = z.J;
        g.dE_jac = z.H;
        CU(rcm_launch_fjac(g, z.q));
        CU(rcm_launch_fdh_newton(fdh_args(z), z.q));
        s->launches += 2;
        return RCM_OK;
    };
    auto start = [&](Slot& z, int k, int c0) -> int {
        z.c0 = c0;
        z.n = std::min((int)ch, col0 + ncol - c0);
        z.iter = 0;
        z.live = true;
        if (first) CU(cudaMemcpyAsync(z.Ttau, s->d_T + (size_t)c0 * NLAY, z.n * NLAY * D, cudaMemcpyDeviceToDevice, z.q));
        CU(cudaMemcpyAsync(z.ntrop, ntrop + (c0 - col0), z.n * sizeof(int), cudaMemcpyHostToDevice, z.q));
        if ((st = diag_prep(s, z.q, c0, z.n, z.T, z.Tprev, z.vmr, z.stat, z.tile, nullptr, z.a)) != RCM_OK) return st;
        if ((st = evaluate(z, z.Ed0, z.Eu0, z.dE0)) != RCM_OK) return st;
        if (vmr_scale) {
            CU(rcm_launch_diag_scale(z.tile, z.a.ntiles, sc, z.q));
            s->launches += 1;
        }
        return check(z, k);
    };
    auto download = [&](const Slot& z) -> int {
        const size_t r = (size_t)(z.c0 - col0);
        if (F) CU(cudaMemcpyAsync(F + r * 4, z.F, z.n * 4 * D, cudaMemcpyDeviceToHost, z.q));
        if (dT_adj) CU(cudaMemcpyAsync(dT_adj + r * NLAY, z.dT, z.n * NLAY * D, cudaMemcpyDeviceToHost, z.q));
        if (E_down) CU(cudaMemcpyAsync(E_down + r * NLEV, z.Edo, z.n * NLEV * D, cudaMemcpyDeviceToHost, z.q));
        if (E_up) CU(cudaMemcpyAsync(E_up + r * NLEV, z.Euo, z.n * NLEV * D, cudaMemcpyDeviceToHost, z.q));
        if (iters) CU(cudaMemcpyAsync(iters + r, z.iters, z.n * sizeof(int), cudaMemcpyDeviceToHost, z.q));
        return RCM_OK;
    };
    int next = col0;
    for (int k = 0; k < 2 && next < col0 + ncol; ++k, next += (int)ch)
        if ((st = start(slot[k], k, next)) != RCM_OK) return st;
    for (int k = 0; slot[0].live || slot[1].live; k ^= 1) {
        Slot& z = slot[k];
        if (!z.live) continue;
        CU(cudaStreamSynchronize(z.q));
        if (s->h_fdh_count[k] > 0) {
            if ((st = newton(z)) != RCM_OK) return st;
            ++z.iter;
            if ((st = check(z, k)) != RCM_OK) return st;
            continue;
        }
        if ((st = download(z)) != RCM_OK) return st;
        z.live = false;
        if (next < col0 + ncol) {
            if ((st = start(z, k, next)) != RCM_OK) return st;
            next += (int)ch;
        }
    }
    return diag_end(s);
}

namespace {
struct CkptArray { void* dev; size_t bytes; };

int ckpt_arrays(rcm_solver* s, CkptArray* out, bool col_solar, bool col_cloud) {
    const size_t n = (size_t)s->ncol, D = sizeof(double);
    int k = 0;
    out[k++] = {s->d_T, n * NLAY * D};
    out[k++] = {s->d_Ts, n * D};
    out[k++] = {s->d_vmr, n * s->nactive * NLAY * D};
    out[k++] = {s->d_rh, n * NLAY * D};
    out[k++] = {s->d_Tprev, n * NLAY * D};
    out[k++] = {s->d_time, n * sizeof(float)};
    out[k++] = {s->d_dt, n * D};
    out[k++] = {s->d_Ed, n * NLEV * D};
    out[k++] = {s->d_Eu, n * NLEV * D};
    out[k++] = {s->d_dE, n * NLAY * D};
    if (col_solar) out[k++] = {s->d_solar_col, n * D};
    if (col_cloud) out[k++] = {s->d_cloud_col, n * D};
    return k;
}
}

int rcm_column_count(const rcm_solver* s) { return s ? s->ncol : 0; }

int rcm_save_checkpoint(rcm_solver* s, const char* path) {
    if (!s || !path) return RCM_ERR_ARG;
    if (s->ncol <= 0) return fail(s, RCM_ERR_STATE, "no columns loaded");
    CU(cudaSetDevice(s->device));
    CU(cudaStreamSynchronize(s->stream));
    FILE* f = std::fopen(path, "wb");
    if (!f) return fail(s, RCM_ERR_IO, std::string("cannot write ") + path);
    const long long hdr[8] = {s->ncol, s->nactive, (long long)s->p.species_mask, s->step_index, s->has_col_solar ? 1 : 0,
                              s->has_col_cloud ? 1 : 0, s->lbl_mode ? 1 : 0, s->dc.nwvl};
    bool ok = std::fwrite("RCMCKPT1", 1, 8, f) == 8 && std::fwrite(hdr, sizeof(hdr), 1, f) == 1 &&
              std::fwrite(s->plevel, sizeof(s->plevel), 1, f) == 1;
    CkptArray arr[12];
    const int na = ckpt_arrays(s, arr, s->has_col_solar, s->has_col_cloud);
    std::vector<char> buf;
    for (int k = 0; k < na && ok; ++k) {
        buf.resize(arr[k].bytes);
        cudaError_t e = cudaMemcpy(buf.data(), arr[k].dev, arr[k].bytes, cudaMemcpyDeviceToHost);
        if (e != cudaSuccess) {
            std::fclose(f);
            return cuda_fail(s, e, "checkpoint download");
        }
        ok = std::fwrite(buf.data(), 1, arr[k].bytes, f) == arr[k].bytes;
    }
    ok = (std::fclose(f) == 0) && ok;
    return ok ? RCM_OK : fail(s, RCM_ERR_IO, std::string("short write to ") + path);
}

int rcm_load_checkpoint(rcm_solver* s, const char* path) {
    if (!s || !path) return RCM_ERR_ARG;
    CU(cudaSetDevice(s->device));
    CU(cudaStreamSynchronize(s->stream));
    FILE* f = std::fopen(path, "rb");
    if (!f) return fail(s, RCM_ERR_IO, std::string("cannot read ") + path);
    char magic[8];
    long long hdr[8];
    double plevel[RCM_NLEVEL];
    if (std::fread(magic, 1, 8, f) != 8 || std::memcmp(magic, "RCMCKPT1", 8) != 0 || std::fread(hdr, sizeof(hdr), 1, f) != 1 ||
        std::fread(plevel, sizeof(plevel), 1, f) != 1 || hdr[0] <= 0 || hdr[0] > (1LL << 30)) {
        std::fclose(f);
        return fail(s, RCM_ERR_FORMAT, std::string(path) + " is not a checkpoint of this solver");
    }
    set_active_species(s);
    if ((unsigned)hdr[2] != s->p.species_mask || (int)hdr[1] != s->nactive) {
        std::fclose(f);
        return fail(s, RCM_ERR_STATE, "checkpoint was written with another species_mask");
    }
    if ((hdr[6] != 0) != s->lbl_mode) {
        std::fclose(f);
        return fail(s, RCM_ERR_STATE, "checkpoint belongs to the other spectral path (repwvl / line-by-line)");
    }
    if (hdr[7] != 0 && (s->has_table || s->lbl_mode) && hdr[7] != s->dc.nwvl) {
        std::fclose(f);
        return fail(s, RCM_ERR_STATE, "checkpoint was written with a table of another wavelength count");
    }
    int st = ensure_columns(s, (int)hdr[0]);
    if (st != RCM_OK) {
        std::fclose(f);
        return st;
    }
    s->ncol = (int)hdr[0];
    if ((hdr[4] || hdr[5]) && !s->d_solar_col) {
        cudaError_t e = dalloc(s->d_solar_col, (size_t)s->cap);
        if (e == cudaSuccess) e = dalloc(s->d_cloud_col, (size_t)s->cap);
        if (e != cudaSuccess) {
            std::fclose(f);
            s->ncol = 0;
            return cuda_fail(s, e, "checkpoint: per-column forcing buffers");
        }
    }
    CkptArray arr[12];
    const int na = ckpt_arrays(s, arr, hdr[4] != 0, hdr[5] != 0);
    std::vector<char> buf;
    for (int k = 0; k < na; ++k) {
        buf.resize(arr[k].bytes);
        if (std::fread(buf.data(), 1, arr[k].bytes, f) != arr[k].bytes) {
            std::fclose(f);
            s->ncol = 0;
            return fail(s, RCM_ERR_FORMAT, std::string(path) + " is truncated");
        }
        cudaError_t e = cudaMemcpy(arr[k].dev, buf.data(), arr[k].bytes, cudaMemcpyHostToDevice);
        if (e != cudaSuccess) {
            std::fclose(f);
            s->ncol = 0;
            return cuda_fail(s, e, "checkpoint upload");
        }
    }
    std::fclose(f);
    if (!s->has_plevel || std::memcmp(s->plevel, plevel, sizeof(plevel)) != 0) s->coef_dirty = true;
    std::memcpy(s->plevel, plevel, sizeof(plevel));
    s->has_plevel = true;
    s->const_dirty = true;
    s->step_index = (long)hdr[3];
    s->has_col_solar = hdr[4] != 0;
    s->has_col_cloud = hdr[5] != 0;
    s->tau_valid = false;
    s->tile_vmr_valid = false;
    return RCM_OK;
}

int rcm_step_host(rcm_solver* s, const double* Tlayer_in, const double* Tsurf_in, const double* vmr_active_in,
                  double* E_down, double* E_up, double* dE, double* Tlayer_out, double* Tsurf_out) {
    if (!s) return RCM_ERR_ARG;
    int max_chunks = 8;
    if (const char* e = std::getenv("RCM_PIPE_CHUNKS")) max_chunks = std::max(1, std::min(16, std::atoi(e)));
    const int nchunk = (s && !s->lbl_mode && s->has_table) ? std::min(max_chunks, s->ncol / 4096) : 0;
    if (nchunk < 2) {
        int st = rcm_update_columns(s, Tlayer_in, Tsurf_in, vmr_active_in);
        if (st != RCM_OK) return st;
        st = rcm_advance_async(s, 1, nullptr);
        if (st != RCM_OK) return st;
        return rcm_get_state(s, Tlayer_out, Tsurf_out, nullptr, nullptr, E_down, E_up, dE, nullptr);
    }
    CU(cudaSetDevice(s->device));
    int st = ensure_diag(s, 1);
    if (st != RCM_OK) return st;
    st = refresh_const(s);
    if (st != RCM_OK) return st;
    if (!s->pipe_stream[0]) {
        for (int i = 0; i < 3; ++i) {
            CU(cudaStreamCreateWithFlags(&s->pipe_stream[i], cudaStreamNonBlocking));
            CU(cudaEventCreateWithFlags(&s->pipe_done[i], cudaEventDisableTiming));
        }
        CU(cudaEventCreateWithFlags(&s->pipe_start, cudaEventDisableTiming));
    }
    if (use_split(s))
        return step_host_split(s, nchunk, Tlayer_in, Tsurf_in, vmr_active_in, E_down, E_up, dE, Tlayer_out, Tsurf_out);
    const int nsm = nsm_of(s);
    Part whole[2];
    plan_parts(s, s->ncol, nsm, whole);
    const int C = whole[0].sh.C;
    const int per = ((s->ncol + nchunk - 1) / nchunk + C - 1) / C * C;
    CU(cudaEventRecord(s->pipe_start, s->stream));
    for (int i = 0; i < 3; ++i) CU(cudaStreamWaitEvent(s->pipe_stream[i], s->pipe_start, 0));
    const size_t D = sizeof(double);
    const int na = s->nactive;
    for (int k = 0, c0 = 0; c0 < s->ncol; ++k, c0 += per) {
        const int n = std::min(per, s->ncol - c0);
        const size_t o = (size_t)c0;
        cudaStream_t q = s->pipe_stream[k % 3];
        if (Tlayer_in) CU(cudaMemcpyAsync(s->d_T + o * NLAY, Tlayer_in + o * NLAY, n * NLAY * D, cudaMemcpyHostToDevice, q));
        if (Tsurf_in) CU(cudaMemcpyAsync(s->d_Ts + o, Tsurf_in + o, n * D, cudaMemcpyHostToDevice, q));
        if (vmr_active_in)
            CU(cudaMemcpyAsync(s->d_vmr + o * na * NLAY, vmr_active_in + o * na * NLAY, (size_t)n * na * NLAY * D,
                               cudaMemcpyHostToDevice, q));
        const Part p{c0, n, whole[0].sh};
        st = launch_part(s, MODE_STEP, 1, true, p, nsm, q);
        if (st != RCM_OK) return st;
        if (E_down) CU(cudaMemcpyAsync(E_down + o * NLEV, s->d_Ed + o * NLEV, n * NLEV * D, cudaMemcpyDeviceToHost, q));
        if (E_up) CU(cudaMemcpyAsync(E_up + o * NLEV, s->d_Eu + o * NLEV, n * NLEV * D, cudaMemcpyDeviceToHost, q));
        if (dE) CU(cudaMemcpyAsync(dE + o * NLAY, s->d_dE + o * NLAY, n * NLAY * D, cudaMemcpyDeviceToHost, q));
        if (Tlayer_out) CU(cudaMemcpyAsync(Tlayer_out + o * NLAY, s->d_T + o * NLAY, n * NLAY * D, cudaMemcpyDeviceToHost, q));
        if (Tsurf_out) CU(cudaMemcpyAsync(Tsurf_out + o, s->d_Ts + o, n * D, cudaMemcpyDeviceToHost, q));
    }
    for (int i = 0; i < 3; ++i) {
        CU(cudaEventRecord(s->pipe_done[i], s->pipe_stream[i]));
        CU(cudaStreamWaitEvent(s->stream, s->pipe_done[i], 0));
    }
    CU(rcm_launch_reduce_diag(s->d_diag, 1, s->ncol, s->p.dT_converged, s->d_red, s->d_ticket, s->d_scalars, s->stream));
    s->launches += 1;
    s->step_index += 1;
    s->tau_valid = false;
    CU(cudaStreamSynchronize(s->stream));
    return RCM_OK;
}

int rcm_cplkavg_device(rcm_solver* s, int n, const double* lo_nm, const double* hi_nm, const double* t, double* out) {
    if (!s || n <= 0 || !lo_nm || !hi_nm || !t || !out) return RCM_ERR_ARG;
    CU(cudaSetDevice(s->device));
    double* d = nullptr;
    CU(dalloc(d, (size_t)4 * n));
    cudaError_t e = cudaMemcpyAsync(d, lo_nm, n * sizeof(double), cudaMemcpyHostToDevice, s->stream);
    if (e == cudaSuccess) e = cudaMemcpyAsync(d + n, hi_nm, n * sizeof(double), cudaMemcpyHostToDevice, s->stream);
    if (e == cudaSuccess) e = cudaMemcpyAsync(d + 2 * (size_t)n, t, n * sizeof(double), cudaMemcpyHostToDevice, s->stream);
    if (e == cudaSuccess) e = rcm_launch_cplkavg(n, d, d + n, d + 2 * (size_t)n, d + 3 * (size_t)n, s->d_exp_tab, s->opt_cplk_narrow, s->stream);
    if (e == cudaSuccess) e = cudaMemcpyAsync(out, d + 3 * (size_t)n, n * sizeof(double), cudaMemcpyDeviceToHost, s->stream);
    if (e == cudaSuccess) e = cudaStreamSynchronize(s->stream);
    cudaFree(d);
    if (e != cudaSuccess) return cuda_fail(s, e, "cplkavg");
    s->launches += 1;
    return RCM_OK;
}

long rcm_launch_count(const rcm_solver* s) { return s ? s->launches : 0; }

int rcm_host_graph_stats(const rcm_solver* s, long* captures, long* replays) {
    if (!s || !captures || !replays) return RCM_ERR_ARG;
    *captures = s->hg.captures;
    *replays = s->hg.replays;
    return RCM_OK;
}

int rcm_fp64_microbench(rcm_solver* s, int which, double* gops) {
    if (!s || !gops || which < 0 || which > 3) return RCM_ERR_ARG;
    CU(cudaSetDevice(s->device));
    int nsm = 148;
    cudaDeviceGetAttribute(&nsm, cudaDevAttrMultiProcessorCount, s->device);
    const int grid = nsm * 8;
    const long iters = (which == 0) ? 40000 : 4000;
    double* d = nullptr;
    CU(dalloc(d, (size_t)grid * 256));
    cudaEvent_t e0, e1;
    cudaEventCreate(&e0);
    cudaEventCreate(&e1);
    cudaError_t e = rcm_launch_microbench(which, d, s->d_exp_tab, iters / 10, grid, s->stream);
    float best = 1e30f;
    for (int rep = 0; rep < 3 && e == cudaSuccess; ++rep) {
        cudaEventRecord(e0, s->stream);
        e = rcm_launch_microbench(which, d, s->d_exp_tab, iters, grid, s->stream);
        cudaEventRecord(e1, s->stream);
        if (e == cudaSuccess) e = cudaEventSynchronize(e1);
        float ms = 0;
        cudaEventElapsedTime(&ms, e0, e1);
        if (ms < best) best = ms;
    }
    cudaEventDestroy(e0);
    cudaEventDestroy(e1);
    cudaFree(d);
    if (e != cudaSuccess) return cuda_fail(s, e, "microbench");
    s->launches += 4;
    *gops = (double)grid * 256.0 * 8.0 * (double)iters / (best * 1e-3) / 1e9;
    return RCM_OK;
}

int rcm_kernel_time_ms(rcm_solver* s, int reset, double* avg_ms, long* n_launches) {
    if (!s) return RCM_ERR_ARG;
    CU(cudaSetDevice(s->device));
    CU(cudaStreamSynchronize(s->stream));
    for (auto& ev : s->ev_used) {
        float ms = 0;
        if (cudaEventElapsedTime(&ms, ev.first, ev.second) == cudaSuccess) {
            s->kt_ms += ms;
            s->kt_n += 1;
        }
        s->ev_free.push_back(ev);
    }
    s->ev_used.clear();
    if (avg_ms) *avg_ms = s->kt_n ? s->kt_ms / s->kt_n : 0.0;
    if (n_launches) *n_launches = s->kt_n;
    if (reset) {
        s->kt_ms = 0.0;
        s->kt_n = 0;
    }
    return RCM_OK;
}

}
```

### our_first_climate_model_b200/csrc/rcm_kernels.cuh

```cuda
#ifndef RCM_KERNELS_CUH
#define RCM_KERNELS_CUH

#include <cuda_runtime.h>

#include "rcm_internal.h"

constexpr int NLAY = RCM_NLAYER;
constexpr int NLEV = RCM_NLEVEL;
constexpr int MAX_ANGLE = 64;
constexpr int MAX_TPERT = 16;
constexpr int PLK_MAX = 128;
constexpr int MAX_PAIR = 16;
constexpr int HALF = NLAY / 2;
constexpr int RCM_LBL_C = 16, RCM_LBL_NT = 128;
#ifndef RCM_EXP_LOG2
#define RCM_EXP_LOG2 10
#endif
constexpr int EXP_LOG2 = RCM_EXP_LOG2, EXP_TAB = 1 << EXP_LOG2;
constexpr int EXP_REP = (EXP_LOG2 == 7) ? 8 : 1;
#ifdef RCM_EXP_DEG_OVERRIDE
constexpr int EXP_DEG = RCM_EXP_DEG_OVERRIDE;
#else
constexpr int EXP_DEG = (EXP_LOG2 == 7) ? 3 : 2;
#endif
static_assert(EXP_LOG2 == 7 || EXP_LOG2 == 10, "exp table configurations: 128 x 8 copies or 1024 x 1");
constexpr double EXP_L2E = EXP_TAB * 1.4426950408889634;

struct DevConst {
    int nwvl, nangle, nactive, n_tpert, n_species, n_p;
    int species[RCM_NSPECIES];
    int cloud_layer;
    double cloud_tau, dp, max_dT, dt_cap, solar_irr, dT_converged;
    int ip[NLAY];
    int ipcell[NLAY];
    int cloud_row;
    double cloud_w[NLAY];
    double delP[NLAY], numDens[NLAY], tref_ip[NLAY], player[NLAY], conv[NLAY];
    double t_pert[MAX_TPERT];
    int nslot, nchain;
    int chain_len[MAX_ANGLE + 2];
    double neg_inv_mu_l2e[MAX_ANGLE + 2];
    double cmu[MAX_ANGLE + 2];
    double csum;
    int npair;
    int pair_type[MAX_PAIR];
    int pair_lenA[MAX_PAIR], pair_lenB[MAX_PAIR];
    double pair_nim[MAX_PAIR + 1];
    double expc[4];
};

struct StepArgs {
    int ncol;
    int diag_ncol;
    int C;
    int nthreads;
    int stage_rows;
    int clampk;
    double tau_clamp;
    double T_floor;
    int ntiles;
    int nsteps;
    long step_index;
    const double* __restrict__ coef;
    const double* __restrict__ planck_c;
    const double* __restrict__ planck_k;
    double* Tlayer;
    double* Tsurf;
    double* vmr;
    const double* rel_hum;
    double* Tprev;
    float* time_h;
    double* E_down;
    double* E_up;
    double* dE;
    double* dt;
    double* diag;
    double* tau_io;
    int* lowpos_t;
    const double* exp_tab;
    int h2o_slot;
    const double* solar_col;
    const double* cloud_col;
};

struct LblArgs {
    int ncol, ntiles, nwvl, nchunks, chunk_len, nact, h2o_slot, o3_slot;
    int clampk;
    long step_index;
    double co2_factor, tau_clamp;
    const double* __restrict__ wvl_lo;
    const double* __restrict__ wvl_hi;
    const double* __restrict__ wn_hi;
    const double* __restrict__ wn_lo;
    const int* __restrict__ bin_ok;
    const double* __restrict__ tau3;
    const double* __restrict__ h2o_ref;
    const double* __restrict__ o3_ref;
    const double* __restrict__ exp_tab;
    double* Tlayer; double* Tsurf; double* vmr; const double* rel_hum; double* Tprev; float* time_h;
    double* sH; double* sO; double* dTstat;
    double* part;
    double* E_down; double* E_up; double* dE; double* dt; double* diag;
    const double* solar_col; const double* cloud_col;
};

struct SplitArgs {
    int ncol;
    int diag_ncol;
    int ntiles, nsplit, ipu, nitem, nunits;
    int stage_rows, clampk, h2o_slot;
    double tau_clamp, T_floor;
    const double* __restrict__ coef;
    const double* __restrict__ planck_c;
    const double* __restrict__ planck_k;
    const double* __restrict__ exp_tab;
    double* Tlayer; double* Tsurf; double* vmr; const double* rel_hum; double* Tprev; float* time_h;
    double* E_down; double* E_up; double* dE; double* dt; double* diag;
    const double* solar_col; const double* cloud_col;
    unsigned char* tile;
    double* part;
    double* dTstat;
    unsigned* counter;
    int quota;
};
struct SplitColFlags {
    int finish;
    int prep;
    int first;
    int write_all_vmr;
    int write_out;
    int diag_step;
};
struct SplitMultiArgs {
    int nsteps;
    unsigned* done;
    unsigned* ready;
};
size_t rcm_split_tile_bytes();
size_t rcm_split_part_doubles();
int rcm_split_ipu();
cudaError_t rcm_launch_split_col(const SplitArgs& a, const SplitColFlags& f, cudaStream_t st);
cudaError_t rcm_launch_split_rt(const SplitArgs& a, int grid, cudaStream_t st);
cudaError_t rcm_launch_split_multi(const SplitArgs& a, const SplitMultiArgs& m, int grid, cudaStream_t st);

enum { MODE_STEP = 0, MODE_TAU = 1, MODE_RT = 2 };

size_t rcm_step_smem_bytes(int C, int nactive, int nthreads);
cudaError_t rcm_upload_const(const DevConst& c);
cudaError_t rcm_launch_step(int mode, const StepArgs& a, int nactive, int grid, cudaStream_t st);
size_t rcm_reduce_scratch_doubles(int nsteps);
cudaError_t rcm_launch_reduce_diag(const double* diag, int nsteps, int ncol, double dT_converged, double* scratch,
                                   unsigned* ticket, double* scalars, cudaStream_t st);
cudaError_t rcm_launch_coef(const double* xsec_file, double* coef, int nt, int ns, int nw, int np, int nact,
                            const int* d_species, cudaStream_t st);
cudaError_t rcm_launch_coef3(const double* coef4, double* coef3, size_t nrows, cudaStream_t st);
cudaError_t rcm_launch_microbench(int which, double* out, const double* tab, long iters, int grid,
                                  cudaStream_t st);
size_t rcm_lbl_smem_bytes(int C, int nthreads);
cudaError_t rcm_launch_lbl_step(const LblArgs& a, cudaStream_t st, cudaEvent_t ev0, cudaEvent_t ev1);
struct SolarArgs {
    int n, doublings;
    double tau_s, mu_s, g_asym, albedo, daytime, E_0;
    const double* tau_s_col; const double* mu_s_col; const double* albedo_col;
    double* solar_irr; double* r_total; double* cloud_tau;
};
cudaError_t rcm_launch_solar(const SolarArgs& a, cudaStream_t st);
cudaError_t rcm_launch_cplkavg(int n, const double* lo, const double* hi, const double* t, double* out,
                               const double* exp_tab, int narrow, cudaStream_t st);

#endif
```

### our_first_climate_model_b200/csrc/rcm_split_kernels.cuh

```cuda
#pragma once

constexpr int SPLIT_C = 16, SPLIT_NT = 128, SPLIT_G = 4;
constexpr int SPLIT_IPU = 5;
constexpr int SPLIT_COL_NT = 128;

constexpr int TB_INVT = 0;
constexpr int TB_DELT = TB_INVT + TBD_LEN;
constexpr int TB_DTDP = TB_DELT + TBD_LEN;
constexpr int TB_VMR = TB_DTDP + TBD_LEN;
constexpr int TB_INVTS = TB_VMR + 5 * TBD_LEN;
constexpr int TB_CLOUD = TB_INVTS + SPLIT_C;
constexpr int TB_DOUBLES = TB_CLOUD + SPLIT_C;
constexpr int TBI_IT = 0;
constexpr int TBI_ROWSEL = TBI_IT + TBI_LEN;
constexpr int TBI_ROWOFF = TBI_ROWSEL + TBI_LEN;
constexpr int TBI_OUTSIDE = TBI_ROWOFF + NLAY * NCAND;
constexpr int TB_INTS = (TBI_OUTSIDE + 1 + 3) / 4 * 4;
constexpr int TILE_BYTES = TB_DOUBLES * 8 + TB_INTS * 4;
static_assert(TILE_BYTES % 16 == 0, "bulk copies move multiples of 16 bytes");
constexpr int ROWB3 = 16 * 8;
constexpr int ROWS3 = ROWB3 + 16;
constexpr int ROWBUF3 = NLAY * NCAND * ROWS3;
constexpr int SPLIT_PART = 2 * NLEV * SPLIT_C;

struct SplitColSmem {
    double sT[NLAY * SPLIT_C], sTh[NLAY * SPLIT_C], sPrev[NLAY * SPLIT_C], sRh[NLAY * SPLIT_C], sEd[NLEV * SPLIT_C],
        sEu[NLEV * SPLIT_C], sdE[NLAY * SPLIT_C], sdt[SPLIT_C], sTs[SPLIT_C], sSol[SPLIT_C], sStat[SPLIT_C];
    int sit[NLAY * SPLIT_C], sitmin[NLAY], sout[NLAY + 1];
};

template <bool STANDALONE>
__device__ __forceinline__ void split_col_body(const SplitArgs& a, const SplitColFlags f, const int tile, SplitColSmem& cs) {
    constexpr int C = SPLIT_C, NT = SPLIT_COL_NT, LC = NLAY * C;
    double* const sT = cs.sT; double* const sTh = cs.sTh; double* const sPrev = cs.sPrev; double* const sRh = cs.sRh;
    double* const sEd = cs.sEd; double* const sEu = cs.sEu; double* const sdE = cs.sdE; double* const sdt = cs.sdt;
    double* const sTs = cs.sTs; double* const sSol = cs.sSol; double* const sStat = cs.sStat;
    int* const sit = cs.sit; int* const sitmin = cs.sitmin; int* const sout = cs.sout;
    int extrap = 0;
    const int tid = threadIdx.x;
    const int col0 = tile * C, ncl = min(C, a.ncol - col0);
    const int nact = cst.nactive, nwvl = cst.nwvl;
    if (STANDALONE && tile == 0 && tid == 0 && a.counter) *a.counter = 0u;
    double* const tb = reinterpret_cast<double*>(a.tile + (size_t)tile * TILE_BYTES);
    int* const tbi = reinterpret_cast<int*>(tb + TB_DOUBLES);
    const bool feedback = f.prep && !f.first && a.h2o_slot >= 0;
    for (int i = tid; i < LC; i += NT) {
        const int cc = i / NLAY, l = i % NLAY;
        const size_t gi = (size_t)(col0 + (cc < ncl ? cc : 0)) * NLAY + l;
        sT[l * C + cc] = __ldcg(a.Tlayer + gi);
        if (f.prep) sPrev[l * C + cc] = __ldcg(a.Tprev + gi);
        if (feedback) sRh[l * C + cc] = a.rel_hum[gi];
    }
    if (tid < C) {
        const int col = col0 + (tid < ncl ? tid : 0);
        sTs[tid] = __ldcg(a.Tsurf + col);
        sSol[tid] = a.solar_col ? a.solar_col[col] : cst.solar_irr;
        if (f.finish) sStat[tid] = __ldcg(a.dTstat + col);
    }
    if (f.finish) {
        const double* part = a.part + (size_t)tile * a.nsplit * SPLIT_PART;
        for (int i = tid; i < SPLIT_PART; i += NT) {
            const int row = i / C;
            double sum = 0.0;
            if (row != NLAY)
                for (int sp = 0; sp < a.nsplit; ++sp) sum += __ldcg(part + (size_t)sp * SPLIT_PART + i);
            if (row < NLAY) sEd[i + C] = sum;
            else if (row == NLAY) sEd[i % C] = 0.0;
            else sEu[i - NLEV * C] = sum;
        }
    }
    __syncthreads();

    if (f.finish) {
        for (int i = tid; i < LC; i += NT) {
            const int l = i / C, cc = i % C;
            double d = sEd[l * C + cc] - sEd[(l + 1) * C + cc] + sEu[(l + 1) * C + cc] - sEu[l * C + cc];
            if (l == NLAY - 1) d += sSol[cc] + sEd[NLAY * C + cc] - sEu[NLAY * C + cc];
            sdE[i] = d;
        }
        __syncthreads();
        if (tid < C) {
            double mx = sdE[tid], mabs = 0.0;
#pragma unroll
            for (int l = 0; l < NLAY; ++l) {
                const double d = sdE[l * C + tid];
                if (mx < d) mx = d;
                mabs = fmax(mabs, fabs(d));
            }
            double dt = (double)(float)cst.max_dT / mx * (1004.0 * cst.dp * 100.0) / 9.80665;
            if (dt > cst.dt_cap) dt = cst.dt_cap;
            sdt[tid] = dt;
            if (tid < ncl) {
                const int col = col0 + tid;
                a.time_h[col] = __ldcg(a.time_h + col) + (float)dt / 3600;
                if (a.diag) {
                    double* dg = a.diag + ((size_t)f.diag_step * a.diag_ncol + col) * 4;
                    dg[0] = sSol[tid] - sEu[tid];
                    dg[1] = sStat[tid];
                    dg[2] = mabs;
                    dg[3] = dt;
                }
                if (f.write_out) a.dt[col] = dt;
            }
        }
        __syncthreads();
        for (int i = tid; i < LC; i += NT) {
            const int l = i / C, cc = i % C;
            const double Tn = sT[i] + sdE[i] * sdt[cc] * 9.80665 / (1004.0 * cst.dp * 100.0);
            sT[i] = Tn;
            if (l == NLAY - 1) {
                const double ts = Tn * cst.conv[NLAY - 1];
                sTs[cc] = ts;
                if (cc < ncl) a.Tsurf[col0 + cc] = ts;
            }
        }
        if (f.write_out) {
            for (int i = tid; i < NLEV * ncl; i += NT) {
                const int cc = i / NLEV, l = i % NLEV;
                a.E_down[(size_t)col0 * NLEV + i] = sEd[l * C + cc];
                a.E_up[(size_t)col0 * NLEV + i] = sEu[l * C + cc];
            }
            for (int i = tid; i < NLAY * ncl; i += NT) a.dE[(size_t)col0 * NLAY + i] = sdE[(i % NLAY) * C + i / NLAY];
        }
        __syncthreads();
        if (!f.prep) {
            for (int i = tid; i < NLAY * ncl; i += NT) a.Tlayer[(size_t)col0 * NLAY + i] = sT[(i % NLAY) * C + i / NLAY];
            return;
        }
    }

    auto indices = [&] {
        for (int i = tid; i < LC; i += NT) {
            const int l = i / C, cc = i % C, r = prow(l);
            const double midT = sT[i], tref = cst.tref_ip[r];
            const int it = lowerpos_t(tref, midT, cst.n_tpert);
            const double t0 = tref + cst.t_pert[it], t1 = tref + cst.t_pert[it + 1];
            extrap |= (midT < tref + cst.t_pert[0]) | (midT > tref + cst.t_pert[cst.n_tpert - 1]);
            sit[r * C + cc] = it;
            tbi[TBI_IT + tbix(r, cc)] = it;
            const double dT = (midT - t0) / (t1 - t0);
            tb[TB_DELT + tbd(r, cc)] = dT;
            tb[TB_DTDP + tbd(r, cc)] = __dmul_rn(dT, cst.delP[r]);
        }
    };
    if (f.first) indices();
    for (int i = tid; i < LC; i += NT) sTh[i] = sT[i] * cst.conv[i / C];
    __syncthreads();
    for (int i = tid; i < LC; i += NT) {
        const int l = i / C, cc = i % C;
        const double my = sTh[i];
        int rank = 0;
#pragma unroll
        for (int l2 = 0; l2 < NLAY; ++l2) {
            const double v = sTh[l2 * C + cc];
            rank += (v > my || (v == my && l2 < l)) ? 1 : 0;
        }
        const double Tn = my / cst.conv[rank];
        sT[rank * C + cc] = Tn;
        sdE[rank * C + cc] = fabs(Tn - sPrev[rank * C + cc]);
    }
    __syncthreads();
    for (int i = tid; i < NLAY * ncl; i += NT) {
        const double v = sT[(i % NLAY) * C + i / NLAY];
        a.Tlayer[(size_t)col0 * NLAY + i] = v;
        a.Tprev[(size_t)col0 * NLAY + i] = v;
    }
    if (tid < ncl) {
        double dmax = 0.0;
#pragma unroll
        for (int l = 0; l < NLAY; ++l) dmax = fmax(dmax, sdE[l * C + tid]);
        a.dTstat[col0 + tid] = dmax;
    }
    for (int i = tid; i < nact * LC; i += NT) {
        const int cc = i % C, l = (i / C) % NLAY, sp = i / LC;
        const bool h2o = (sp == a.h2o_slot) && !f.first;
        if (!h2o && !f.write_all_vmr) continue;
        double v = 0.0;
        if (cc < ncl) {
            const size_t gi = ((size_t)(col0 + cc) * nact + sp) * NLAY + l;
            if (h2o) {
                const double Tc = sT[l * C + cc] - 273.15;
                const double e_sat = 6.1094 * exp(17.625 * Tc / (Tc + 243.04));
                v = sRh[l * C + cc] * e_sat / cst.player[l];
                a.vmr[gi] = v;
            } else {
                v = a.vmr[gi];
            }
        }
        tb[TB_VMR + sp * TBD_LEN + tbd(prow(l), cc)] = v;
    }
    if (!f.first) indices();
    for (int i = tid; i < LC; i += NT) tb[TB_INVT + tbd(prow(i / C), i % C)] = (1.0 / fmax(sT[i], a.T_floor)) * L2E64;
    if (tid < C) {
        tb[TB_INVTS + tid] = (1.0 / fmax(sTs[tid], a.T_floor)) * L2E64;
        tb[TB_CLOUD + tid] = a.cloud_col ? a.cloud_col[col0 + (tid < ncl ? tid : 0)] : cst.cloud_tau;
    }
    const int any_extrap = __syncthreads_or(extrap);
    if (tid < NLAY) {
        int mn = sit[tid * C], mx = mn;
        for (int cc = 1; cc < C; ++cc) {
            mn = min(mn, sit[tid * C + cc]);
            mx = max(mx, sit[tid * C + cc]);
        }
        sitmin[tid] = mn;
        sout[tid] = (mx - mn >= NCAND);
        for (int k = 0; k < NCAND; ++k) tbi[TBI_ROWOFF + NCAND * tid + k] = (cst.ipcell[tid] + min(mn + k, cst.n_tpert - 2)) * nwvl * ROWB3;
    }
    __syncthreads();
    for (int i = tid; i < LC; i += NT) {
        const int r = i / C;
        tbi[TBI_ROWSEL + tbix(r, i % C)] = (NCAND * r + min(sit[i] - sitmin[r], NCAND - 1)) * ROWS3;
    }
    if (tid == 0) {
        int any = any_extrap;
        for (int r = 0; r < NLAY; ++r) any |= sout[r];
        tbi[TBI_OUTSIDE] = any;
    }
}

__device__ __noinline__ void split_col_body_call(const SplitArgs& a, const SplitColFlags f, const int tile, SplitColSmem& cs) {
    split_col_body<false>(a, f, tile, cs);
}

__global__ void __launch_bounds__(SPLIT_COL_NT, 8) rcm_split_col_kernel(const SplitArgs a, const SplitColFlags f) {
    __shared__ SplitColSmem cs;
    split_col_body<true>(a, f, blockIdx.x, cs);
}

__device__ __forceinline__ unsigned ld_acquire_gpu(const unsigned* p) {
    unsigned v;
    asm volatile("ld.acquire.gpu.global.u32 %0, [%1];" : "=r"(v) : "l"(p) : "memory");
    return v;
}
__device__ __forceinline__ void st_release_gpu(unsigned* p, unsigned v) {
    asm volatile("st.release.gpu.global.u32 [%0], %1;" ::"l"(p), "r"(v) : "memory");
}

__device__ __noinline__ void wait_tile_ready(const unsigned* flag, unsigned step) {
    unsigned spins = 0;
    while (ld_acquire_gpu(flag) < step) {
        __nanosleep(128);
        if (++spins > (1u << 23)) __trap();
    }
    asm volatile("fence.proxy.async;" ::: "memory");
}

__device__ __forceinline__ void mbar_init(unsigned mbar, unsigned count) {
    asm volatile("mbarrier.init.shared::cta.b64 [%0], %1;" ::"r"(mbar), "r"(count) : "memory");
    asm volatile("fence.mbarrier_init.release.cluster;" ::: "memory");
}
__device__ __forceinline__ void tma_load_1d(unsigned dst, const void* src, unsigned bytes, unsigned mbar) {
    asm volatile("fence.proxy.async.shared::cta;" ::: "memory");
    asm volatile("mbarrier.arrive.expect_tx.shared::cta.b64 _, [%0], %1;" ::"r"(mbar), "r"(bytes) : "memory");
    asm volatile("cp.async.bulk.shared::cluster.global.mbarrier::complete_tx::bytes [%0], [%1], %2, [%3];" ::"r"(dst), "l"(src),
                 "r"(bytes), "r"(mbar)
                 : "memory");
}
__device__ __forceinline__ void mbar_wait(unsigned mbar, unsigned phase) {
    asm volatile(
        "{\n\t.reg .pred p;\n\t"
        "WAIT_%=:\n\t"
        "mbarrier.try_wait.parity.shared::cta.b64 p, [%0], %1;\n\t"
        "@p bra DONE_%=;\n\t"
        "bra WAIT_%=;\n\t"
        "DONE_%=:\n\t}" ::"r"(mbar),
        "r"(phase)
        : "memory");
}

constexpr size_t SPLIT_SMEM = (size_t)EXP_TAB * EXP_REP * 8 + (size_t)SPLIT_G * ROWBUF3 + TILE_BYTES + 2 * PLK_MAX * 8 + 48;
static_assert(SPLIT_PART * 8 <= ROWBUF3, "a warp's row buffer carries its partial fluxes after the wavelength loop");

static_assert(sizeof(SplitColSmem) <= (size_t)SPLIT_G * ROWBUF3, "the K5 body of the multi-step kernel works in the row buffers");
static_assert(SPLIT_COL_NT == SPLIT_NT, "the multi-step kernel runs the K5 body with its own CTA");

template <bool CLAMPK>
__global__ void __launch_bounds__(SPLIT_NT, 3) rcm_split_rt_kernel(const SplitArgs a) {
#define RCM_SPLIT_MULTI 0
#include "rcm_split_unit_loop.inc"
#undef RCM_SPLIT_MULTI
}

template <bool CLAMPK>
__global__ void __launch_bounds__(SPLIT_NT, 3) rcm_split_multi_kernel(const __grid_constant__ SplitArgs a, const __grid_constant__ SplitMultiArgs m) {
#define RCM_SPLIT_MULTI 1
#include "rcm_split_unit_loop.inc"
#undef RCM_SPLIT_MULTI
}
```

### our_first_climate_model_b200/csrc/rcm_split_unit_loop.inc

```
    constexpr int C = SPLIT_C, NT = SPLIT_NT, G = SPLIT_G, NACT = 5;
    extern __shared__ __align__(128) unsigned char smem_raw[];
    double* const s_exp = reinterpret_cast<double*>(smem_raw);
    unsigned char* const s_rows = smem_raw + (size_t)EXP_TAB * EXP_REP * 8;
    double* const tb = reinterpret_cast<double*>(s_rows + (size_t)G * ROWBUF3);
    const int* const tbi = reinterpret_cast<const int*>(tb + TB_DOUBLES);
    double* const s_plk = reinterpret_cast<double*>(reinterpret_cast<unsigned char*>(tb) + TILE_BYTES);
    unsigned long long* const s_mbar = reinterpret_cast<unsigned long long*>(s_plk + 2 * PLK_MAX);
    volatile int* const s_next = reinterpret_cast<volatile int*>(s_mbar + 1);

    const int tid = threadIdx.x, lane = tid & 31, warp = tid >> 5;
    const int h = tid & 1, q = tid >> 1, c = q % C, g = q / C;
    const int sb = tbd(h * HALF, c), sbi = tbix(h * HALF, c);
    const int nwvl = cst.nwvl;
    for (int i = tid; i < EXP_TAB * EXP_REP; i += NT) s_exp[i] = a.exp_tab[i / EXP_REP];
    const unsigned tab_lane = (unsigned)__cvta_generic_to_shared(s_exp + (lane & (EXP_REP - 1)));
    const bool plk_smem = nwvl <= PLK_MAX;
    if (plk_smem)
        for (int i = tid; i < nwvl; i += NT) {
            s_plk[i] = a.planck_c[i];
            s_plk[PLK_MAX + i] = a.planck_k[i];
        }
    const unsigned mbar = (unsigned)__cvta_generic_to_shared(s_mbar);
    const unsigned tb_addr = (unsigned)__cvta_generic_to_shared(tb);
    unsigned char* const rows = s_rows + (size_t)warp * ROWBUF3;
    const unsigned rows_addr = (unsigned)__cvta_generic_to_shared(rows);
#if RCM_SPLIT_MULTI
    auto fetch_block = [&](int u) {
        const int tile_u = (u % a.nunits) / a.nsplit;
        const bool ready = ld_acquire_gpu(m.ready + tile_u) >= (unsigned)(u / a.nunits);
        s_next[2] = !ready;
        if (!ready) return;
        asm volatile("fence.proxy.async;" ::: "memory");
        tma_load_1d(tb_addr, a.tile + (size_t)tile_u * TILE_BYTES, TILE_BYTES, mbar);
    };
    if (tid == 0) {
        mbar_init(mbar, 1);
        const int u = (int)atomicAdd(a.counter, 1u);
        s_next[0] = u;
        s_next[1] = 1;
        s_next[2] = 0;
        if (u < a.nunits * m.nsteps) fetch_block(u);
    }
#else
    if (tid == 0) {
        mbar_init(mbar, 1);
        const int u = (int)atomicAdd(a.counter, 1u);
        s_next[0] = u;
        s_next[1] = 1;
        if (u < a.nunits) tma_load_1d(tb_addr, a.tile + (size_t)(u / a.nsplit) * TILE_BYTES, TILE_BYTES, mbar);
    }
#endif
    __syncthreads();
    int unit = *s_next;
    unsigned phase = 0;

    auto request_rows = [&](int w) {
        __syncwarp();
        const char* base = reinterpret_cast<const char*>(a.coef) + (size_t)w * ROWB3 + (lane & 7) * 16;
        const unsigned dst0 = rows_addr + (lane & 7) * 16 + (lane >> 3) * ROWS3;
        const int* ro = tbi + TBI_ROWOFF + (lane >> 3);
        unsigned off[NCAND * NLAY / 4];
#pragma unroll
        for (int i = 0; i < NCAND * NLAY / 4; ++i) off[i] = (unsigned)ro[4 * i];
#pragma unroll
        for (int i = 0; i < NCAND * NLAY / 4; ++i) cp_async16(dst0 + 4 * i * ROWS3, base + off[i]);
        cp_async_commit();
    };
    auto tau_from = [&](int j, const double2* cf, double cl) -> double {
        const int r = h * HALF + j;
        const double dT = tb[TB_DELT + sb + j * C], dTdP = tb[TB_DTDP + sb + j * C];
        double c[16];
#pragma unroll
        for (int q2 = 0; q2 < 8; ++q2) {
            const double2 v = cf[q2];
            c[2 * q2] = v.x;
            c[2 * q2 + 1] = v.y;
        }
        double acc = 0.0;
#pragma unroll
        for (int k = 0; k < NACT; ++k) {
            double v = fma(c[3 * k + 1], dT, c[3 * k]);
            v = fma(c[3 * k + 2], dTdP, v);
            acc = fma(v, tb[TB_VMR + k * TBD_LEN + sb + j * C], acc);
        }
        acc = acc * cst.numDens[r];
        return fma(cst.cloud_w[r], cl, acc);
    };

    const int tau_clamp_hi = __double2hiint(a.tau_clamp);
#if RCM_SPLIT_MULTI
    while (unit < a.nunits * m.nsteps) {
        const int step = unit / a.nunits, unit_s = unit - step * a.nunits;
        const int tile = unit_s / a.nsplit, split = unit_s - tile * a.nsplit;
        if (tid == 0) {
            s_next[4] = tile;
            s_next[5] = step;
            s_next[6] = unit_s;
        }
#else
    while (unit < a.nunits) {
        const int tile = unit / a.nsplit, split = unit - tile * a.nsplit;
#endif
        mbar_wait(mbar, phase);
        phase ^= 1u;
        const bool staged = a.stage_rows && !tbi[TBI_OUTSIDE];
        const int item0 = split * a.ipu, item1 = min(item0 + a.ipu, a.nitem);
        double E1[HALF], E2[HALF], Eu20 = 0.0;
#pragma unroll
        for (int j = 0; j < HALF; ++j) E1[j] = E2[j] = 0.0;
        if (staged) request_rows(min(g + item0 * G, nwvl - 1));
#pragma unroll 1
        for (int item = item0; item < item1; ++item) {
            const int w_any = g + item * G;
            const bool real = w_any < nwvl;
            const int w = real ? w_any : nwvl - 1;
            double tau[HALF], Bo[HALF];
            const double cl = tb[TB_CLOUD + c];
            if (staged) {
                cp_async_wait_all();
                __syncwarp();
#pragma unroll
                for (int j = 0; j < HALF; ++j) {
                    const double v = tau_from(j, reinterpret_cast<const double2*>(rows + tbi[TBI_ROWSEL + sbi + j * C]), cl);
                    tau[j] = CLAMPK ? v : clamp_hi(v, tau_clamp_hi);
                }
                if (item + 1 < item1) request_rows(min(w_any + G, nwvl - 1));
            } else {
#pragma unroll
                for (int j = 0; j < HALF; ++j) {
                    const int cell = cst.ipcell[h * HALF + j] + tbi[TBI_IT + sbi + j * C];
                    const double v = tau_from(j, reinterpret_cast<const double2*>(a.coef) + (size_t)(cell * nwvl + w) * 8, cl);
                    tau[j] = fmax(CLAMPK ? v : clamp_hi(v, tau_clamp_hi), TAU_FLOOR);
                }
            }
            const double pc = plk_smem ? s_plk[w] : __ldg(a.planck_c + w);
            const double pk = !real ? 0.0 : plk_smem ? s_plk[PLK_MAX + w] : __ldg(a.planck_k + w);
#pragma unroll
            for (int j = 0; j < HALF; ++j)
                Bo[j] = div_fast(pk, exp_scaled<false>(pc, tb[TB_INVT + sb + j * C], tab_lane) - 1.0);
            const double Bs = div_fast(pk, exp_scaled<false>(pc, tb[TB_INVTS + c], tab_lane) - 1.0);
            sweep_item<CLAMPK>(tau, Bo, Bs, h, tab_lane, E1, E2, Eu20);
        }
        {
            double* part = reinterpret_cast<double*>(s_rows + (size_t)g * ROWBUF3);
#pragma unroll
            for (int j = 0; j < HALF; ++j) {
                const int l = h ? (NLAY - 1 - j) : j;
                part[l * C + c] = h ? E2[j] : E1[j];
                part[(NLEV + l) * C + c] = h ? E1[j] : E2[j];
            }
            if (h) part[(NLEV + NLAY) * C + c] = Eu20;
        }
        __syncthreads();
        if (tid == 0) {
            const int taken = s_next[1];
#if RCM_SPLIT_MULTI
            const int u = (int)atomicAdd(a.counter, 1u);
            s_next[0] = u;
            s_next[1] = taken + 1;
            if (u < a.nunits * m.nsteps) fetch_block(u);
        }
        double* out = a.part + (size_t)s_next[6] * SPLIT_PART;
#else
            const int u = (taken < a.quota) ? (int)atomicAdd(a.counter, 1u) : a.nunits;
            s_next[0] = u;
            s_next[1] = taken + 1;
            if (u < a.nunits) tma_load_1d(tb_addr, a.tile + (size_t)(u / a.nsplit) * TILE_BYTES, TILE_BYTES, mbar);
        }
        double* out = a.part + (size_t)unit * SPLIT_PART;
#endif
        for (int i = tid; i < SPLIT_PART; i += NT) {
            double sum = 0.0;
            if (i / C != NLAY) {
#pragma unroll
                for (int gg = 0; gg < G; ++gg) sum += reinterpret_cast<const double*>(s_rows + (size_t)gg * ROWBUF3)[i];
            }
            out[i] = sum;
        }
#if RCM_SPLIT_MULTI
        {
            __threadfence();
            __syncthreads();
            const int tile_e = s_next[4], step_e = s_next[5];
            if (tid == 0) {
                const unsigned before = atomicAdd(m.done + tile_e, 1u);
                s_next[3] = ((before + 1u) % (unsigned)a.nsplit) == 0u;
            }
            __syncthreads();
            if (s_next[3]) {
                __threadfence();
                SplitColFlags f;
                f.finish = 1;
                f.prep = (step_e + 1 < m.nsteps);
                f.first = 0;
                f.write_all_vmr = 0;
                f.write_out = (step_e + 1 == m.nsteps);
                f.diag_step = step_e;
                split_col_body_call(a, f, tile_e, *reinterpret_cast<SplitColSmem*>(s_rows));
                __threadfence();
                __syncthreads();
                if (tid == 0) st_release_gpu(m.ready + tile_e, (unsigned)(step_e + 1));
            }
            if (tid == 0 && s_next[2]) {
                const int u = s_next[0], tile_u = (u % a.nunits) / a.nsplit;
                wait_tile_ready(m.ready + tile_u, (unsigned)(u / a.nunits));
                tma_load_1d(tb_addr, a.tile + (size_t)tile_u * TILE_BYTES, TILE_BYTES, mbar);
            }
        }
#endif
        __syncthreads();
        unit = *s_next;
    }
```

Measured before the change: 40.20 billion.

## Prepare next step's tile inside finish kernel to skip per-call prep launch

When nsteps==1, the finish column kernel now also runs the next step's prep phase (convective adjustment, H2O feedback, tile indices) and stores the pending temperatures and water vapour in new Tnext/h2o_next buffers. The next call can then skip the separate prep launch and swap buffers, guarded by a generation counter that every state-mutating API call invalidates. The change also pads the shared-memory column stride to reduce bank conflicts, has each thread rank up to three layers in the sort, caches time_h, and restricts the vmr loop to the species range that is actually written. It adds extra global traffic and bookkeeping, and wrong results if any state change misses an invalidation.

Result: no change. 40.54 billion (median of 6 runs) (+0.8%).

```diff
diff --git a/our_first_climate_model_b200/csrc/rcm_capi.cu b/our_first_climate_model_b200/csrc/rcm_capi.cu
--- a/our_first_climate_model_b200/csrc/rcm_capi.cu
+++ b/our_first_climate_model_b200/csrc/rcm_capi.cu
@@ -66,6 +66,9 @@
     int opt_multi = 1;
     size_t tile_cap = 0, spart_cap = 0;
     bool tile_vmr_valid = false;
+    double *d_Tnext = nullptr, *d_h2o_next = nullptr;
+    long state_gen = 0;
+    long prepared_gen = -1;
     std::vector<double> stage;
     std::string err;
     long launches = 0;
@@ -103,6 +106,8 @@
 int cuda_fail(rcm_solver* s, cudaError_t e, const char* what) {
     return fail(s, RCM_ERR_CUDA, std::string(what) + ": " + cudaGetErrorString(e));
 }
+
+void invalidate_prepared(rcm_solver* s) { s->state_gen += 1; }
 
 #define CU(call)                                          \
     do {                                                  \
@@ -256,6 +261,7 @@
         g_const_owner[dev] = s;
     }
     if (!s->const_dirty) return RCM_OK;
+    invalidate_prepared(s);
     CU(cudaStreamSynchronize(s->stream));
     DevConst& d = s->dc;
     set_active_species(s);
@@ -337,6 +343,11 @@
     s->tile_vmr_valid = false;
     if (s->d_dTstat) cudaFree(s->d_dTstat);
     s->d_dTstat = nullptr;
+    for (double** p : {&s->d_Tnext, &s->d_h2o_next}) {
+        if (*p) cudaFree(*p);
+        *p = nullptr;
+    }
+    invalidate_prepared(s);
     if (s->d_solar_col) cudaFree(s->d_solar_col);
     if (s->d_cloud_col) cudaFree(s->d_cloud_col);
     s->d_solar_col = s->d_cloud_col = nullptr;
@@ -464,6 +475,7 @@
         CU(dalloc(s->d_tile, tiles * rcm_split_tile_bytes()));
         s->tile_cap = tiles;
         s->tile_vmr_valid = false;
+        invalidate_prepared(s);
     }
     if (need_part > s->spart_cap || !s->d_spart) {
         CU(dalloc(s->d_spart, need_part));
@@ -476,6 +488,8 @@
         s->multi_cap = tiles;
     }
     if (!s->d_dTstat) CU(dalloc(s->d_dTstat, (size_t)s->cap));
+    if (!s->d_Tnext) CU(dalloc(s->d_Tnext, (size_t)s->cap * NLAY));
+    if (!s->d_h2o_next) CU(dalloc(s->d_h2o_next, (size_t)s->cap * NLAY));
     if (!s->d_counter) {
         CU(dalloc(s->d_counter, (size_t)4));
         CU(cudaMemsetAsync(s->d_counter, 0, 4 * sizeof(unsigned), s->stream));
@@ -521,6 +535,8 @@
     a.dTstat = s->d_dTstat + o;
     a.counter = s->d_counter + which;
     a.quota = 1 << 30;
+    a.Tnext = s->d_Tnext + o * NLAY;
+    a.h2o_next = s->d_h2o_next + o * NLAY;
     return a;
 }
 
@@ -566,23 +582,32 @@
     st = ensure_split(s);
     if (st != RCM_OK) return st;
     const int nsm = nsm_of(s);
-    const SplitArgs a = split_args(s, 0, s->ncol, 0);
-    SplitColFlags f{};
-    f.prep = 1;
-    f.first = (s->step_index == 0);
-    f.write_all_vmr = !s->tile_vmr_valid;
-    CU(rcm_launch_split_col(a, f, s->stream));
-    s->launches += 1;
-    s->tile_vmr_valid = true;
     static const int multi_rounds = std::getenv("RCM_MULTI_ROUNDS") ? std::atoi(std::getenv("RCM_MULTI_ROUNDS")) : 24;
+    SplitArgs a = split_args(s, 0, s->ncol, 0);
     const int grid1 = split_grid(s, a, nsm);
     const bool few_rounds = a.nunits < (long long)multi_rounds * grid1;
     const bool fits = (long long)a.nunits * nsteps + 2LL * grid1 < (1LL << 31);
-    if (nsteps >= 2 && fits && (s->opt_multi == 2 || (s->opt_multi == 1 && few_rounds))) {
+    const bool multi = nsteps >= 2 && fits && (s->opt_multi == 2 || (s->opt_multi == 1 && few_rounds));
+    const bool prepared = s->prepared_gen == s->state_gen && s->step_index > 0 && s->tile_vmr_valid && (nsteps == 1 || multi);
+    s->prepared_gen = -1;
+    if (prepared) {
+        std::swap(s->d_Tprev, s->d_Tnext);
+        std::swap(a.Tprev, a.Tnext);
+    } else {
+        SplitColFlags f{};
+        f.prep = 1;
+        f.first = (s->step_index == 0);
+        f.write_all_vmr = !s->tile_vmr_valid;
+        CU(rcm_launch_split_col(a, f, s->stream));
+        s->launches += 1;
+        s->tile_vmr_valid = true;
+    }
+    if (multi) {
         SplitMultiArgs m{};
         m.nsteps = nsteps;
         m.done = s->d_multi;
         m.ready = s->d_multi + a.ntiles;
+        m.prepared = prepared;
         CU(cudaMemsetAsync(s->d_multi, 0, 2 * (size_t)a.ntiles * sizeof(unsigned), s->stream));
         SplitArgs am = a;
         am.quota = 1 << 30;
@@ -595,13 +620,16 @@
         if (st != RCM_OK) return st;
         SplitColFlags e{};
         e.finish = 1;
-        e.prep = (k + 1 < nsteps);
+        e.ahead = (nsteps == 1);
+        e.prep = (k + 1 < nsteps) || e.ahead;
         e.first = 0;
         e.write_out = (k + 1 == nsteps);
         e.diag_step = k;
+        e.prepared = (k == 0) && prepared;
         CU(rcm_launch_split_col(a, e, s->stream));
         s->launches += 1;
     }
+    if (nsteps == 1) s->prepared_gen = s->state_gen;
     return RCM_OK;
 }
 
@@ -842,7 +870,8 @@
     void* ptrs[] = {s->d_coef3, s->d_xsec_file, s->d_coef, s->d_species, s->d_planck_c, s->d_planck_k, s->d_exp_tab, s->d_T, s->d_Ts, s->d_vmr, s->d_rh,
                     s->d_Tprev, s->d_time, s->d_lbl_lo, s->d_lbl_hi, s->d_lbl_tau5, s->d_lbl_h2o_ref, s->d_lbl_o3_ref, s->d_sH, s->d_sO,
                     s->d_dTstat, s->d_part, s->d_Ed, s->d_Eu, s->d_dE, s->d_dt, s->d_diag, s->d_scalars, s->d_red, s->d_tau,
-                    s->d_lowpos, s->d_solar_col, s->d_cloud_col, s->d_ticket, s->d_tile, s->d_spart, s->d_counter, s->d_multi, s->d_diagnose};
+                    s->d_lowpos, s->d_solar_col, s->d_cloud_col, s->d_ticket, s->d_tile, s->d_spart, s->d_counter, s->d_multi, s->d_diagnose,
+                    s->d_Tnext, s->d_h2o_next};
     for (void* q : ptrs)
         if (q) cudaFree(q);
     for (auto& e : s->ev_free) { cudaEventDestroy(e.first); cudaEventDestroy(e.second); }
@@ -876,6 +905,7 @@
 int rcm_set_params(rcm_solver* s, const rcm_params* p) {
     if (!s || !p) return RCM_ERR_ARG;
     if (p->nangle < 1 || p->nangle > MAX_ANGLE || p->cloud_layer >= RCM_NLAYER) return fail(s, RCM_ERR_ARG, "bad params");
+    invalidate_prepared(s);
     unsigned old = s->p.species_mask;
     s->p = *p;
     if (old != p->species_mask) {
@@ -889,6 +919,7 @@
 
 int rcm_set_option(rcm_solver* s, int option, int value) {
     if (!s) return RCM_ERR_ARG;
+    invalidate_prepared(s);
     if (option == 0) {
         s->opt_angle_cubes = value ? 1 : 0;
         s->const_dirty = true;
@@ -926,6 +957,7 @@
 
 int rcm_set_stream(rcm_solver* s, void* cuda_stream) {
     if (!s) return RCM_ERR_ARG;
+    invalidate_prepared(s);
     s->stream = cuda_stream ? (cudaStream_t)cuda_stream : s->own_stream;
     return RCM_OK;
 }
@@ -943,6 +975,7 @@
     if (!s || !xsec || !wvl || !weight || !p_grid || !t_ref || !t_pert) return RCM_ERR_ARG;
     if (n_tpert < 2 || n_tpert > MAX_TPERT || n_species != RCM_NSPECIES || n_wvl < 1 || n_p < 2)
         return fail(s, RCM_ERR_ARG, "unsupported table dimensions");
+    invalidate_prepared(s);
     CU(cudaSetDevice(s->device));
     const size_t n = (size_t)n_tpert * n_species * n_wvl * n_p;
     CU(dalloc(s->d_xsec_file, n));
@@ -970,6 +1003,7 @@
 
 int rcm_set_spectral_grid(rcm_solver* s, const double* wvl, const double* weight, int n_wvl) {
     if (!s || !wvl || !weight || n_wvl < 1) return RCM_ERR_ARG;
+    invalidate_prepared(s);
     CU(cudaSetDevice(s->device));
     const double h = 6.62607e-34, c = 299792458, kB = 1.380649e-23;
     std::vector<double> pc(n_wvl), pk(n_wvl);
@@ -1013,6 +1047,7 @@
     if (!s || !wvl || !tau5 || nwvl < 2 || !h2o_ref) return RCM_ERR_ARG;
     for (int i = 1; i < nwvl; ++i)
         if (!(wvl[i] > wvl[i - 1])) return fail(s, RCM_ERR_ARG, "LBL wavelengths must be strictly ascending");
+    invalidate_prepared(s);
     CU(cudaSetDevice(s->device));
     std::vector<double> lo(nwvl), hi(nwvl);
     for (int i = 0; i < nwvl; ++i) {
@@ -1069,6 +1104,7 @@
 int rcm_set_columns(rcm_solver* s, int ncol, const double* plevel_hPa, const double* Tlayer, const double* Tsurf,
                     const double* vmr9, const double* rel_hum) {
     if (!s || ncol <= 0 || !plevel_hPa || !Tlayer || !Tsurf || !vmr9 || !rel_hum) return RCM_ERR_ARG;
+    invalidate_prepared(s);
     CU(cudaSetDevice(s->device));
     int st = ensure_columns(s, ncol);
     if (st != RCM_OK) return st;
@@ -1102,6 +1138,7 @@
                          const double* albedo, int cloud_from_tau_s, double* solar_irr_out, double* r_total_out) {
     if (!s) return RCM_ERR_ARG;
     if (s->ncol <= 0) return fail(s, RCM_ERR_STATE, "rcm_set_columns first");
+    invalidate_prepared(s);
     CU(cudaSetDevice(s->device));
     if (!sp) {
         s->has_col_solar = s->has_col_cloud = false;
@@ -1157,6 +1194,7 @@
 int rcm_update_columns(rcm_solver* s, const double* Tlayer, const double* Tsurf, const double* vmr_active) {
     if (!s) return RCM_ERR_ARG;
     if (s->ncol <= 0) return fail(s, RCM_ERR_STATE, "rcm_set_columns first");
+    invalidate_prepared(s);
     CU(cudaSetDevice(s->device));
     const size_t n = (size_t)s->ncol;
     if (Tlayer) CU(cudaMemcpyAsync(s->d_T, Tlayer, n * NLAY * sizeof(double), cudaMemcpyHostToDevice, s->stream));
@@ -1170,6 +1208,7 @@
 
 int rcm_set_step_index(rcm_solver* s, long step_index) {
     if (!s || step_index < 0) return RCM_ERR_ARG;
+    invalidate_prepared(s);
     s->step_index = step_index;
     return RCM_OK;
 }
@@ -1289,6 +1328,7 @@
     CU(cudaSetDevice(s->device));
     int st = ensure_diag(s, nsteps);
     if (st != RCM_OK) return st;
+    if (!use_split(s)) invalidate_prepared(s);
     if (s->lbl_mode) {
         st = lbl_advance(s, nsteps);
         if (st != RCM_OK) return st;
@@ -1882,6 +1922,7 @@
 
 int rcm_load_checkpoint(rcm_solver* s, const char* path) {
     if (!s || !path) return RCM_ERR_ARG;
+    invalidate_prepared(s);
     CU(cudaSetDevice(s->device));
     CU(cudaStreamSynchronize(s->stream));
     FILE* f = std::fopen(path, "rb");
@@ -1955,6 +1996,7 @@
 int rcm_step_host(rcm_solver* s, const double* Tlayer_in, const double* Tsurf_in, const double* vmr_active_in,
                   double* E_down, double* E_up, double* dE, double* Tlayer_out, double* Tsurf_out) {
     if (!s) return RCM_ERR_ARG;
+    invalidate_prepared(s);
     int max_chunks = 8;
     if (const char* e = std::getenv("RCM_PIPE_CHUNKS")) max_chunks = std::max(1, std::min(16, std::atoi(e)));
     const int nchunk = (s && !s->lbl_mode && s->has_table) ? std::min(max_chunks, s->ncol / 4096) : 0;
diff --git a/our_first_climate_model_b200/csrc/rcm_kernels.cuh b/our_first_climate_model_b200/csrc/rcm_kernels.cuh
--- a/our_first_climate_model_b200/csrc/rcm_kernels.cuh
+++ b/our_first_climate_model_b200/csrc/rcm_kernels.cuh
@@ -122,6 +122,8 @@
     double* dTstat;
     unsigned* counter;
     int quota;
+    double* Tnext;
+    double* h2o_next;
 };
 struct SplitColFlags {
     int finish;
@@ -130,11 +132,14 @@
     int write_all_vmr;
     int write_out;
     int diag_step;
+    int ahead;
+    int prepared;
 };
 struct SplitMultiArgs {
     int nsteps;
     unsigned* done;
     unsigned* ready;
+    int prepared;
 };
 size_t rcm_split_tile_bytes();
 size_t rcm_split_part_doubles();
diff --git a/our_first_climate_model_b200/csrc/rcm_split_kernels.cuh b/our_first_climate_model_b200/csrc/rcm_split_kernels.cuh
--- a/our_first_climate_model_b200/csrc/rcm_split_kernels.cuh
+++ b/our_first_climate_model_b200/csrc/rcm_split_kernels.cuh
@@ -23,19 +23,21 @@
 constexpr int ROWBUF3 = NLAY * NCAND * ROWS3;
 constexpr int SPLIT_PART = 2 * NLEV * SPLIT_C;
 
+constexpr int SPLIT_CP = SPLIT_C + 1;
 struct SplitColSmem {
-    double sT[NLAY * SPLIT_C], sTh[NLAY * SPLIT_C], sPrev[NLAY * SPLIT_C], sRh[NLAY * SPLIT_C], sEd[NLEV * SPLIT_C],
-        sEu[NLEV * SPLIT_C], sdE[NLAY * SPLIT_C], sdt[SPLIT_C], sTs[SPLIT_C], sSol[SPLIT_C], sStat[SPLIT_C];
-    int sit[NLAY * SPLIT_C], sitmin[NLAY], sout[NLAY + 1];
+    double sT[NLAY * SPLIT_CP], sTh[NLAY * SPLIT_CP], sPrev[NLAY * SPLIT_CP], sRh[NLAY * SPLIT_CP], sEd[NLEV * SPLIT_CP],
+        sEu[NLEV * SPLIT_CP], sdE[NLAY * SPLIT_CP], sdt[SPLIT_C], sTs[SPLIT_C], sSol[SPLIT_C], sStat[SPLIT_C];
+    int sit[NLAY * SPLIT_CP], sitmin[NLAY], sout[NLAY + 1];
+    float sTime[SPLIT_C];
 };
 
 template <bool STANDALONE>
 __device__ __forceinline__ void split_col_body(const SplitArgs& a, const SplitColFlags f, const int tile, SplitColSmem& cs) {
-    constexpr int C = SPLIT_C, NT = SPLIT_COL_NT, LC = NLAY * C;
+    constexpr int C = SPLIT_C, P = SPLIT_CP, NT = SPLIT_COL_NT, LC = NLAY * C;
     double* const sT = cs.sT; double* const sTh = cs.sTh; double* const sPrev = cs.sPrev; double* const sRh = cs.sRh;
     double* const sEd = cs.sEd; double* const sEu = cs.sEu; double* const sdE = cs.sdE; double* const sdt = cs.sdt;
     double* const sTs = cs.sTs; double* const sSol = cs.sSol; double* const sStat = cs.sStat;
-    int* const sit = cs.sit; int* const sitmin = cs.sitmin; int* const sout = cs.sout;
+    int* const sit = cs.sit; int* const sitmin = cs.sitmin; int* const sout = cs.sout; float* const sTime = cs.sTime;
     int extrap = 0;
     const int tid = threadIdx.x;
     const int col0 = tile * C, ncl = min(C, a.ncol - col0);
@@ -44,29 +46,32 @@
     double* const tb = reinterpret_cast<double*>(a.tile + (size_t)tile * TILE_BYTES);
     int* const tbi = reinterpret_cast<int*>(tb + TB_DOUBLES);
     const bool feedback = f.prep && !f.first && a.h2o_slot >= 0;
+    const double* const Tin = f.prepared ? a.Tprev : a.Tlayer;
     for (int i = tid; i < LC; i += NT) {
         const int cc = i / NLAY, l = i % NLAY;
         const size_t gi = (size_t)(col0 + (cc < ncl ? cc : 0)) * NLAY + l;
-        sT[l * C + cc] = __ldcg(a.Tlayer + gi);
-        if (f.prep) sPrev[l * C + cc] = __ldcg(a.Tprev + gi);
-        if (feedback) sRh[l * C + cc] = a.rel_hum[gi];
+        sT[l * P + cc] = __ldcg(Tin + gi);
+        if (f.prep) sPrev[l * P + cc] = __ldcg(a.Tprev + gi);
+        if (feedback) sRh[l * P + cc] = a.rel_hum[gi];
+        if (f.prepared && a.h2o_slot >= 0 && cc < ncl) a.vmr[((size_t)(col0 + cc) * nact + a.h2o_slot) * NLAY + l] = __ldcg(a.h2o_next + gi);
     }
     if (tid < C) {
         const int col = col0 + (tid < ncl ? tid : 0);
         sTs[tid] = __ldcg(a.Tsurf + col);
         sSol[tid] = a.solar_col ? a.solar_col[col] : cst.solar_irr;
         if (f.finish) sStat[tid] = __ldcg(a.dTstat + col);
+        if (f.finish && tid < ncl) sTime[tid] = __ldcg(a.time_h + col);
     }
     if (f.finish) {
         const double* part = a.part + (size_t)tile * a.nsplit * SPLIT_PART;
         for (int i = tid; i < SPLIT_PART; i += NT) {
-            const int row = i / C;
+            const int row = i / C, cc = i % C;
             double sum = 0.0;
             if (row != NLAY)
                 for (int sp = 0; sp < a.nsplit; ++sp) sum += __ldcg(part + (size_t)sp * SPLIT_PART + i);
-            if (row < NLAY) sEd[i + C] = sum;
-            else if (row == NLAY) sEd[i % C] = 0.0;
-            else sEu[i - NLEV * C] = sum;
+            if (row < NLAY) sEd[(row + 1) * P + cc] = sum;
+            else if (row == NLAY) sEd[cc] = 0.0;
+            else sEu[(row - NLEV) * P + cc] = sum;
         }
     }
     __syncthreads();
@@ -74,16 +79,16 @@
     if (f.finish) {
         for (int i = tid; i < LC; i += NT) {
             const int l = i / C, cc = i % C;
-            double d = sEd[l * C + cc] - sEd[(l + 1) * C + cc] + sEu[(l + 1) * C + cc] - sEu[l * C + cc];
-            if (l == NLAY - 1) d += sSol[cc] + sEd[NLAY * C + cc] - sEu[NLAY * C + cc];
-            sdE[i] = d;
+            double d = sEd[l * P + cc] - sEd[(l + 1) * P + cc] + sEu[(l + 1) * P + cc] - sEu[l * P + cc];
+            if (l == NLAY - 1) d += sSol[cc] + sEd[NLAY * P + cc] - sEu[NLAY * P + cc];
+            sdE[l * P + cc] = d;
         }
         __syncthreads();
         if (tid < C) {
             double mx = sdE[tid], mabs = 0.0;
 #pragma unroll
             for (int l = 0; l < NLAY; ++l) {
-                const double d = sdE[l * C + tid];
+                const double d = sdE[l * P + tid];
                 if (mx < d) mx = d;
                 mabs = fmax(mabs, fabs(d));
             }
@@ -92,7 +97,7 @@
             sdt[tid] = dt;
             if (tid < ncl) {
                 const int col = col0 + tid;
-                a.time_h[col] = __ldcg(a.time_h + col) + (float)dt / 3600;
+                a.time_h[col] = sTime[tid] + (float)dt / 3600;
                 if (a.diag) {
                     double* dg = a.diag + ((size_t)f.diag_step * a.diag_ncol + col) * 4;
                     dg[0] = sSol[tid] - sEu[tid];
@@ -106,8 +111,8 @@
         __syncthreads();
         for (int i = tid; i < LC; i += NT) {
             const int l = i / C, cc = i % C;
-            const double Tn = sT[i] + sdE[i] * sdt[cc] * 9.80665 / (1004.0 * cst.dp * 100.0);
-            sT[i] = Tn;
+            const double Tn = sT[l * P + cc] + sdE[l * P + cc] * sdt[cc] * 9.80665 / (1004.0 * cst.dp * 100.0);
+            sT[l * P + cc] = Tn;
             if (l == NLAY - 1) {
                 const double ts = Tn * cst.conv[NLAY - 1];
                 sTs[cc] = ts;
@@ -117,26 +122,26 @@
         if (f.write_out) {
             for (int i = tid; i < NLEV * ncl; i += NT) {
                 const int cc = i / NLEV, l = i % NLEV;
-                a.E_down[(size_t)col0 * NLEV + i] = sEd[l * C + cc];
-                a.E_up[(size_t)col0 * NLEV + i] = sEu[l * C + cc];
-            }
-            for (int i = tid; i < NLAY * ncl; i += NT) a.dE[(size_t)col0 * NLAY + i] = sdE[(i % NLAY) * C + i / NLAY];
+                a.E_down[(size_t)col0 * NLEV + i] = sEd[l * P + cc];
+                a.E_up[(size_t)col0 * NLEV + i] = sEu[l * P + cc];
+            }
+            for (int i = tid; i < NLAY * ncl; i += NT) a.dE[(size_t)col0 * NLAY + i] = sdE[(i % NLAY) * P + i / NLAY];
         }
         __syncthreads();
-        if (!f.prep) {
-            for (int i = tid; i < NLAY * ncl; i += NT) a.Tlayer[(size_t)col0 * NLAY + i] = sT[(i % NLAY) * C + i / NLAY];
-            return;
+        if (!f.prep || f.ahead) {
+            for (int i = tid; i < NLAY * ncl; i += NT) a.Tlayer[(size_t)col0 * NLAY + i] = sT[(i % NLAY) * P + i / NLAY];
+            if (!f.prep) return;
         }
     }
 
     auto indices = [&] {
         for (int i = tid; i < LC; i += NT) {
             const int l = i / C, cc = i % C, r = prow(l);
-            const double midT = sT[i], tref = cst.tref_ip[r];
+            const double midT = sT[l * P + cc], tref = cst.tref_ip[r];
             const int it = lowerpos_t(tref, midT, cst.n_tpert);
             const double t0 = tref + cst.t_pert[it], t1 = tref + cst.t_pert[it + 1];
             extrap |= (midT < tref + cst.t_pert[0]) | (midT > tref + cst.t_pert[cst.n_tpert - 1]);
-            sit[r * C + cc] = it;
+            sit[r * P + cc] = it;
             tbi[TBI_IT + tbix(r, cc)] = it;
             const double dT = (midT - t0) / (t1 - t0);
             tb[TB_DELT + tbd(r, cc)] = dT;
@@ -144,34 +149,49 @@
         }
     };
     if (f.first) indices();
-    for (int i = tid; i < LC; i += NT) sTh[i] = sT[i] * cst.conv[i / C];
+    for (int i = tid; i < LC; i += NT) sTh[(i / C) * P + i % C] = sT[(i / C) * P + i % C] * cst.conv[i / C];
     __syncthreads();
-    for (int i = tid; i < LC; i += NT) {
-        const int l = i / C, cc = i % C;
-        const double my = sTh[i];
-        int rank = 0;
+    {
+        static_assert(NT % C == 0 && (NLAY * C + NT - 1) / NT <= 3, "K5 ranking: at most three layers of one column per thread");
+        const int cc = tid % C, l0 = tid / C, ne = (LC - tid + NT - 1) / NT;
+        constexpr int LS = NT / C;
+        double my[3];
+        int rank[3] = {0, 0, 0};
+#pragma unroll
+        for (int k = 0; k < 3; ++k) my[k] = k < ne ? sTh[(l0 + k * LS) * P + cc] : 0.0;
 #pragma unroll
         for (int l2 = 0; l2 < NLAY; ++l2) {
-            const double v = sTh[l2 * C + cc];
-            rank += (v > my || (v == my && l2 < l)) ? 1 : 0;
-        }
-        const double Tn = my / cst.conv[rank];
-        sT[rank * C + cc] = Tn;
-        sdE[rank * C + cc] = fabs(Tn - sPrev[rank * C + cc]);
+            const double v = sTh[l2 * P + cc];
+#pragma unroll
+            for (int k = 0; k < 3; ++k) rank[k] += (v > my[k] || (v == my[k] && l2 < l0 + k * LS)) ? 1 : 0;
+        }
+#pragma unroll
+        for (int k = 0; k < 3; ++k)
+            if (k < ne) {
+                const double Tn = my[k] / cst.conv[rank[k]];
+                sT[rank[k] * P + cc] = Tn;
+                sdE[rank[k] * P + cc] = fabs(Tn - sPrev[rank[k] * P + cc]);
+            }
     }
     __syncthreads();
     for (int i = tid; i < NLAY * ncl; i += NT) {
-        const double v = sT[(i % NLAY) * C + i / NLAY];
-        a.Tlayer[(size_t)col0 * NLAY + i] = v;
-        a.Tprev[(size_t)col0 * NLAY + i] = v;
+        const double v = sT[(i % NLAY) * P + i / NLAY];
+        if (f.ahead) {
+            a.Tnext[(size_t)col0 * NLAY + i] = v;
+        } else {
+            a.Tlayer[(size_t)col0 * NLAY + i] = v;
+            a.Tprev[(size_t)col0 * NLAY + i] = v;
+        }
     }
     if (tid < ncl) {
         double dmax = 0.0;
 #pragma unroll
-        for (int l = 0; l < NLAY; ++l) dmax = fmax(dmax, sdE[l * C + tid]);
+        for (int l = 0; l < NLAY; ++l) dmax = fmax(dmax, sdE[l * P + tid]);
         a.dTstat[col0 + tid] = dmax;
     }
-    for (int i = tid; i < nact * LC; i += NT) {
+    const int sp_lo = f.write_all_vmr ? 0 : (!f.first && a.h2o_slot >= 0) ? a.h2o_slot : nact;
+    const int sp_hi = f.write_all_vmr ? nact : (!f.first && a.h2o_slot >= 0) ? a.h2o_slot + 1 : nact;
+    for (int i = sp_lo * LC + tid; i < sp_hi * LC; i += NT) {
         const int cc = i % C, l = (i / C) % NLAY, sp = i / LC;
         const bool h2o = (sp == a.h2o_slot) && !f.first;
         if (!h2o && !f.write_all_vmr) continue;
@@ -179,10 +199,11 @@
         if (cc < ncl) {
             const size_t gi = ((size_t)(col0 + cc) * nact + sp) * NLAY + l;
             if (h2o) {
-                const double Tc = sT[l * C + cc] - 273.15;
+                const double Tc = sT[l * P + cc] - 273.15;
                 const double e_sat = 6.1094 * exp(17.625 * Tc / (Tc + 243.04));
-                v = sRh[l * C + cc] * e_sat / cst.player[l];
-                a.vmr[gi] = v;
+                v = sRh[l * P + cc] * e_sat / cst.player[l];
+                if (f.ahead) a.h2o_next[(size_t)(col0 + cc) * NLAY + l] = v;
+                else a.vmr[gi] = v;
             } else {
                 v = a.vmr[gi];
             }
@@ -190,17 +211,17 @@
         tb[TB_VMR + sp * TBD_LEN + tbd(prow(l), cc)] = v;
     }
     if (!f.first) indices();
-    for (int i = tid; i < LC; i += NT) tb[TB_INVT + tbd(prow(i / C), i % C)] = (1.0 / fmax(sT[i], a.T_floor)) * L2E64;
+    for (int i = tid; i < LC; i += NT) tb[TB_INVT + tbd(prow(i / C), i % C)] = (1.0 / fmax(sT[(i / C) * P + i % C], a.T_floor)) * L2E64;
     if (tid < C) {
         tb[TB_INVTS + tid] = (1.0 / fmax(sTs[tid], a.T_floor)) * L2E64;
         tb[TB_CLOUD + tid] = a.cloud_col ? a.cloud_col[col0 + (tid < ncl ? tid : 0)] : cst.cloud_tau;
     }
     const int any_extrap = __syncthreads_or(extrap);
     if (tid < NLAY) {
-        int mn = sit[tid * C], mx = mn;
+        int mn = sit[tid * P], mx = mn;
         for (int cc = 1; cc < C; ++cc) {
-            mn = min(mn, sit[tid * C + cc]);
-            mx = max(mx, sit[tid * C + cc]);
+            mn = min(mn, sit[tid * P + cc]);
+            mx = max(mx, sit[tid * P + cc]);
         }
         sitmin[tid] = mn;
         sout[tid] = (mx - mn >= NCAND);
@@ -209,7 +230,7 @@
     __syncthreads();
     for (int i = tid; i < LC; i += NT) {
         const int r = i / C;
-        tbi[TBI_ROWSEL + tbix(r, i % C)] = (NCAND * r + min(sit[i] - sitmin[r], NCAND - 1)) * ROWS3;
+        tbi[TBI_ROWSEL + tbix(r, i % C)] = (NCAND * r + min(sit[r * P + i % C] - sitmin[r], NCAND - 1)) * ROWS3;
     }
     if (tid == 0) {
         int any = any_extrap;
diff --git a/our_first_climate_model_b200/csrc/rcm_split_unit_loop.inc b/our_first_climate_model_b200/csrc/rcm_split_unit_loop.inc
--- a/our_first_climate_model_b200/csrc/rcm_split_unit_loop.inc
+++ b/our_first_climate_model_b200/csrc/rcm_split_unit_loop.inc
@@ -196,6 +196,8 @@
                 f.write_all_vmr = 0;
                 f.write_out = (step_e + 1 == m.nsteps);
                 f.diag_step = step_e;
+                f.ahead = 0;
+                f.prepared = step_e == 0 && m.prepared;
                 split_col_body_call(a, f, tile_e, *reinterpret_cast<SplitColSmem*>(s_rows));
                 __threadfence();
                 __syncthreads();
```
